# kuailehaha/liuzhou

Measured on AMD Instinct MI355X. Metric: self-play positions/sec (fixed sims/move), higher is better.
Workload: dtype f16

## Files before the change

### liuzhou_amd/build.py

```python
from __future__ import annotations

import os
import shutil
import subprocess

PKG = os.path.dirname(os.path.abspath(__file__))
CSRC = os.path.join(PKG, "csrc")
LIB = os.path.join(PKG, "libliuzhou_hip.so")
SOURCES = ("lz_ops.hip", "lz_engine.hip", "lz_net.hip", "lz_net_f32.hip", "lz_train.hip", "lz_search.hip", "lz_symmetry.hip",
           "lz_dedup.hip")
HEADERS = ("lz_rules.h", "lz_soa.h", "lz_symmetry.h", "lz_wave.h", "lz_rng.h", "lz_net_dev.h", "lz_live_index.h", "lz_surprise.h", "lz_tree_dev.h", "lz_dedup.h", os.path.join("..", "..", "include", "liuzhou_hip.h"))


def hipcc_path() -> str:
    for cand in (os.environ.get("HIPCC"), "/opt/rocm/bin/hipcc", shutil.which("hipcc")):
        if cand and os.path.exists(cand):
            return cand
    raise RuntimeError("hipcc not found (expected /opt/rocm/bin/hipcc)")


HOST_LIB = os.path.join(PKG, "libliuzhou_host.so")
HOST_SOURCE = os.path.join(CSRC, "lz_host.cpp")
HOST_SOURCES = (HOST_SOURCE, os.path.join(CSRC, "lz_scalar.cpp"),
                os.path.join(CSRC, "lz_symmetry_host.cpp"),
                os.path.join(CSRC, "lz_dedup_host.cpp"))


def build_host(force: bool = False, verbose: bool = False) -> str:
    deps = list(HOST_SOURCES) + [os.path.join(CSRC, h) for h in HEADERS] + [os.path.join(PKG, "..", "include", "liuzhou_scalar.h")]
    if not force and os.path.exists(HOST_LIB) and all(
            (not os.path.exists(d)) or os.path.getmtime(d) <= os.path.getmtime(HOST_LIB) for d in deps):
        return HOST_LIB
    cxx = os.environ.get("CXX") or shutil.which("g++") or shutil.which("c++")
    if not cxx:
        raise RuntimeError("no host C++ compiler (g++) found for libliuzhou_host.so")
    cmd = [cxx, "-O2", "-std=c++17", "-ffp-contract=off", "-fPIC", "-shared", "-fvisibility=hidden", "-o", HOST_LIB,
           *HOST_SOURCES]
    if verbose:
        print(" ".join(cmd))
    subprocess.check_call(cmd)
    return HOST_LIB


def needs_build() -> bool:
    if not os.path.exists(LIB):
        return True
    t = os.path.getmtime(LIB)
    deps = [os.path.join(CSRC, s) for s in SOURCES if os.path.exists(os.path.join(CSRC, s))]
    deps += [os.path.join(CSRC, h) for h in HEADERS]
    return any(os.path.exists(d) and os.path.getmtime(d) > t for d in deps)


def build_hip(force: bool = False, verbose: bool = False) -> str:
    if not force and not needs_build():
        return LIB
    srcs = [os.path.join(CSRC, s) for s in SOURCES if os.path.exists(os.path.join(CSRC, s))]
    cmd = [hipcc_path(), "--offload-arch=gfx950", "-O3", "-std=c++17", "-ffp-contract=off", "-fPIC", "-shared",
           "-fvisibility=hidden", "-o", LIB] + srcs
    if verbose:
        print(" ".join(cmd))
    subprocess.check_call(cmd)
    return LIB


def build_variant(tag: str, defs, force: bool = True, verbose: bool = False) -> str:
    out = os.path.join(PKG, "_exp", f"liblz_{tag}.so")
    os.makedirs(os.path.dirname(out), exist_ok=True)
    if not force and os.path.exists(out) and os.path.getmtime(out) >= os.path.getmtime(LIB):
        return out
    srcs = [os.path.join(CSRC, s) for s in SOURCES if os.path.exists(os.path.join(CSRC, s))]
    cmd = [hipcc_path(), "--offload-arch=gfx950", "-O3", "-std=c++17", "-ffp-contract=off", "-fPIC", "-shared",
           "-fvisibility=hidden", *[d if d.startswith("-") else "-D" + d for d in defs], "-o", out] + srcs
    if verbose:
        print(" ".join(cmd))
    subprocess.check_call(cmd)
    return out


EXT_SOURCE = os.path.join(CSRC, "v0_core_ext.cpp")
EXT_NAME = "_v0_core_native"


def ext_path() -> str:
    import sysconfig
    return os.path.join(PKG, EXT_NAME + (sysconfig.get_config_var("EXT_SUFFIX") or ".so"))


def build_ext(force: bool = False, verbose: bool = False) -> str:
    out = ext_path()
    deps = [EXT_SOURCE, os.path.join(PKG, "..", "include", "liuzhou_hip.h")]
    if not force and os.path.exists(out) and all(os.path.getmtime(d) <= os.path.getmtime(out) for d in deps):
        return out
    import sysconfig
    import pybind11
    from torch.utils import cpp_extension as ce
    cxx = os.environ.get("CXX") or shutil.which("g++") or shutil.which("c++")
    if not cxx:
        raise RuntimeError("no host C++ compiler (g++) found for the compiled v0_core layer")
    rocm = os.environ.get("ROCM_PATH", "/opt/rocm")
    inc = ["-I" + p for p in ce.include_paths()] + ["-I" + sysconfig.get_paths()["include"], "-I" + pybind11.get_include(),
                                                    "-I" + os.path.join(rocm, "include")]
    libdir = ce.library_paths()[0]
    cmd = [cxx, "-O2", "-std=c++17", "-fPIC", "-shared", "-fvisibility=hidden", "-w", "-D__HIP_PLATFORM_AMD__=1", "-DUSE_ROCM=1",
           "-DTORCH_API_INCLUDE_EXTENSION_H", "-DTORCH_EXTENSION_NAME=" + EXT_NAME, "-D_GLIBCXX_USE_CXX11_ABI=1", *inc,
           "-o", out, EXT_SOURCE, "-L" + libdir, "-Wl,-rpath," + libdir, "-ltorch_python", "-ltorch", "-ltorch_cpu", "-lc10",
           "-lc10_hip", "-ldl", "-lpthread"]
    if verbose:
        print(" ".join(cmd))
    subprocess.check_call(cmd)
    return out


if __name__ == "__main__":
    import sys
    if len(sys.argv) >= 3 and sys.argv[1] == "variant":
        print(build_variant(sys.argv[2], sys.argv[3:], verbose=True))
        sys.exit(0)
    print(build_hip(force=True, verbose=True))
    print(build_host(force=True, verbose=True))
    print(build_ext(force=True, verbose=True))
```

### liuzhou_amd/csrc/lz_engine.hip

```cpp
#include <hip/hip_runtime.h>
#include <hip/amd_detail/amd_hip_unsafe_atomics.h>
#include <math.h>
#include <stdint.h>

#include <mutex>

#include "lz_rng.h"
#include "lz_tree_dev.h"

namespace {

__global__ __launch_bounds__(kBlock) void pack_states_kernel(LzStateSoA s, int64_t B, Packed* __restrict__ out) {
    const int64_t i = (int64_t)blockIdx.x * kBlock + threadIdx.x;
    if (i >= B) return;
    State st;
    st.black = cells_equal(s.board + i * 36, 1);
    st.white = cells_equal(s.board + i * 36, -1);
    st.mb = cells_nonzero(s.marks_black + i * 36);
    st.mw = cells_nonzero(s.marks_white + i * 36);
    st.phase = (int)s.phase[i]; st.player = (int)s.current_player[i];
    st.pm_req = (int)s.pending_marks_required[i]; st.pm_rem = (int)s.pending_marks_remaining[i];
    st.pc_req = (int)s.pending_captures_required[i]; st.pc_rem = (int)s.pending_captures_remaining[i];
    st.forced = (int)s.forced_removals_done[i]; st.move_count = (int)s.move_count[i];
    st.msc = (int)s.moves_since_capture[i];
    out[i] = pack(st);
}

__global__ __launch_bounds__(kBlock) void packed_planes_kernel(const Packed* __restrict__ states, int64_t B,
                                                               float* __restrict__ out) {
    const int lane = lane_id();
    const int64_t g = (int64_t)blockIdx.x * kWavesPerBlock + __builtin_amdgcn_readfirstlane((int)(threadIdx.x >> 6));
    if (g >= B) return;
    const State s = unpack(states[g]);
    const bool blk = s.player == 1;
    const uint64_t own = blk ? s.black : s.white, opp = blk ? s.white : s.black;
    const uint64_t sm = blk ? s.mb : s.mw, om = blk ? s.mw : s.mb;
    float4* orow = reinterpret_cast<float4*>(out + g * 396);
    for (int j = lane; j < 99; j += kWave) {
        const int plane = j / 9, cell0 = (j - plane * 9) * 4;
        uint32_t bits;
        if (plane < 4) {
            const uint64_t src = plane == 0 ? own : plane == 1 ? opp : plane == 2 ? sm : om;
            bits = (uint32_t)(src >> cell0) & 0xFu;
        } else bits = (s.phase == plane - 3) ? 0xFu : 0u;
        orow[j] = make_float4((bits & 1) ? 1.f : 0.f, (bits & 2) ? 1.f : 0.f, (bits & 4) ? 1.f : 0.f, (bits & 8) ? 1.f : 0.f);
    }
}

__global__ __launch_bounds__(kBlock) void tree_begin_kernel(Tree t) {
    const int g = blockIdx.x * kBlock + threadIdx.x;
    if (g >= t.B) return;
    begin_game(t, g);
}


__global__ __launch_bounds__(kBlock) void pos_clear_kernel(int* __restrict__ tab, int64_t n) {
    for (int64_t i = (int64_t)blockIdx.x * kBlock + threadIdx.x; i < n / 4; i += (int64_t)gridDim.x * kBlock)
        reinterpret_cast<int4*>(tab)[i] = make_int4(-1, -1, -1, -1);
}

template <bool FORCED = false, bool GUMBEL = false, bool SOLVER = false, bool SHAPE = false>
__global__ __launch_bounds__(kBlock) void tree_select_kernel(Tree t, ForcedArgs fa, GumbelArgs ga, ShapeArgs sh) {
    const int g = wave_game();
    if (g >= t.B) return;
    tree_select<FORCED, GUMBEL, SOLVER, SHAPE>(t, g, lane_id(), load_root_info(t, g), -1, -1, nullptr, FORCED ? fa.k : 0.0,
                                               fa.count, &ga, GUMBEL, &sh);
}
__global__ __launch_bounds__(kBlock) void gumbel_root_kernel(Tree t, GumbelArgs ga,
                                                             const uint8_t* __restrict__ root_noise) {
    const int g = wave_game();
    if (g >= t.B) return;
    if (root_noise != nullptr && root_noise[g] == 0) return;
    gumbel_root_step(t, g, lane_id(), ga);
}


template <bool IS_ROOT, bool COMPACT = false, bool CAP = false, bool SOLVER = false>
__global__ __launch_bounds__(kBlock) void tree_expand_kernel(Tree t, const float* __restrict__ lp1,
                                                             const float* __restrict__ lp2,
                                                             const float* __restrict__ lpm,
                                                             const float* __restrict__ priors220,
                                                             const float* __restrict__ values,
                                                             const float* __restrict__ noise, int noise_stride,
                                                             float epsilon, int step, CapArrays cap, SolverArgs sv) {
    LZ_EXPAND_SCRATCH(sc);
    const int g = wave_game();
    if (g >= t.B) return;
    ptrdiff_t o = 0;
    if (COMPACT) o = (ptrdiff_t)(t.leaf_kind[g] == kLeafExpand ? t.live_row[g] : 0) - g;
    if (CAP && IS_ROOT && !cap_noise(cap, g)) noise = nullptr;
    tree_expand<IS_ROOT, 0, SOLVER>(t, g, lane_id(), lp1 ? lp1 + o * 36 : nullptr, lp2 ? lp2 + o * 36 : nullptr,
                                    lpm ? lpm + o * 36 : nullptr, priors220 ? priors220 + o * 220 : nullptr, values + o,
                                    noise, noise_stride, epsilon, sc, nullptr, step, nullptr, nullptr, &sv);
}

constexpr int kScanBlock = 1024;
constexpr int kScanUnroll = 8;
__global__ __launch_bounds__(kScanBlock) void tree_live_scan_kernel(Tree t, unsigned long long* __restrict__ count) {
    __shared__ int wave_total[kScanBlock / kWave];
    const int tid = threadIdx.x, lane = tid & (kWave - 1), w = tid / kWave;
    const int rounds = (t.B + kScanBlock - 1) / kScanBlock;
    int cnt = 0;
    for (int r0 = 0; r0 < rounds; r0 += kScanUnroll) {
        int kind[kScanUnroll];
#pragma unroll
        for (int u = 0; u < kScanUnroll; ++u) {
            const int g = (r0 + u) * kScanBlock + tid;
            kind[u] = (r0 + u < rounds && g < t.B) ? t.leaf_kind[g] : kLeafInactive;
        }
#pragma unroll
        for (int u = 0; u < kScanUnroll; ++u) cnt += kind[u] == kLeafExpand ? 1 : 0;
    }
    int incl = cnt;
#pragma unroll
    for (int d = 1; d < kWave; d <<= 1) {
        const int v = __shfl_up(incl, d, kWave);
        if (lane >= d) incl += v;
    }
    if (lane == kWave - 1) wave_total[w] = incl;
    __syncthreads();
    int before = 0, total = 0;
    for (int i = 0; i < kScanBlock / kWave; ++i) { if (i < w) before += wave_total[i]; total += wave_total[i]; }
    int row = before + incl - cnt;
    for (int r0 = 0; r0 < rounds; r0 += kScanUnroll) {
        int kind[kScanUnroll];
        Packed st[kScanUnroll];
#pragma unroll
        for (int u = 0; u < kScanUnroll; ++u) {
            const int g = (r0 + u) * kScanBlock + tid;
            const bool in = r0 + u < rounds && g < t.B;
            kind[u] = in ? t.leaf_kind[g] : kLeafInactive;
            if (in) st[u] = load_state(&t.leaf_state[g]);
        }
#pragma unroll
        for (int u = 0; u < kScanUnroll; ++u) {
            if (kind[u] != kLeafExpand) continue;
            const int g = (r0 + u) * kScanBlock + tid;
            t.live_row[g] = row;
            t.live_state[row] = st[u];
            ++row;
        }
    }
    if (tid == 0) *count = (unsigned long long)total;
}

__global__ __launch_bounds__(kScanBlock) void tree_live_scan_seg_kernel(Tree t, int seg_games, int num_segs,
                                                                        unsigned long long* __restrict__ count,
                                                                        long long* __restrict__ seg_row) {
    __shared__ int wave_total[kScanBlock / kWave];
    const int tid = threadIdx.x, lane = tid & (kWave - 1), w = tid / kWave;
    const int rounds = (seg_games + kScanBlock - 1) / kScanBlock;
    int base = 0, end = 0;
    if (tid == 0) seg_row[0] = 0;
    for (int k = 0; k < num_segs; ++k) {
        const int g0 = k * seg_games;
        int cnt = 0;
        for (int r0 = 0; r0 < rounds; r0 += kScanUnroll) {
            int kind[kScanUnroll];
#pragma unroll
            for (int u = 0; u < kScanUnroll; ++u) {
                const int i = (r0 + u) * kScanBlock + tid;
                kind[u] = (r0 + u < rounds && i < seg_games) ? t.leaf_kind[g0 + i] : kLeafInactive;
            }
#pragma unroll
            for (int u = 0; u < kScanUnroll; ++u) cnt += kind[u] == kLeafExpand ? 1 : 0;
        }
        int incl = cnt;
#pragma unroll
        for (int d = 1; d < kWave; d <<= 1) {
            const int v = __shfl_up(incl, d, kWave);
            if (lane >= d) incl += v;
        }
        if (lane == kWave - 1) wave_total[w] = incl;
        __syncthreads();
        int before = 0, total = 0;
        for (int i = 0; i < kScanBlock / kWave; ++i) { if (i < w) before += wave_total[i]; total += wave_total[i]; }
        __syncthreads();
        int row = base + before + incl - cnt;
        for (int r0 = 0; r0 < rounds; r0 += kScanUnroll) {
            int kind[kScanUnroll];
            Packed st[kScanUnroll];
#pragma unroll
            for (int u = 0; u < kScanUnroll; ++u) {
                const int i = (r0 + u) * kScanBlock + tid;
                const bool in = r0 + u < rounds && i < seg_games;
                kind[u] = in ? t.leaf_kind[g0 + i] : kLeafInactive;
                if (in) st[u] = load_state(&t.leaf_state[g0 + i]);
            }
#pragma unroll
            for (int u = 0; u < kScanUnroll; ++u) {
                if (kind[u] != kLeafExpand) continue;
                const int g = g0 + (r0 + u) * kScanBlock + tid;
                t.live_row[g] = row;
                t.live_state[row] = st[u];
                ++row;
            }
        }
        end = base + total;
        if (tid == 0) seg_row[k + 1] = end;
        base = (end + 15) & ~15;
    }
    if (tid == 0) *count = (unsigned long long)base;
}

template <bool IS_ROOT, bool COMPACT = false, bool CAP = false, bool FORCED = false, bool GUMBEL = false,
          bool SOLVER = false, bool SHAPE = false>
__global__ __launch_bounds__(kBlock) void tree_expand_select_kernel(Tree t, const float* __restrict__ lp1,
                                                                    const float* __restrict__ lp2,
                                                                    const float* __restrict__ lpm,
                                                                    const float* __restrict__ values,
                                                                    const float* __restrict__ noise, int noise_stride,
                                                                    float epsilon, int step, CapArrays cap,
                                                                    ForcedArgs fa, GumbelArgs ga, SolverArgs sv,
                                                                    ShapeArgs sh) {
#ifndef LZ_EXP_NO_TREE_PRIO
    __builtin_amdgcn_s_setprio(3);
#endif
    LZ_EXPAND_SCRATCH(sc);
    const int g = wave_game();
    if (g >= t.B) return;
    const int lane = lane_id();
    RootInfo root;
    ptrdiff_t o = 0;
    if (COMPACT) o = (ptrdiff_t)(t.leaf_kind[g] == kLeafExpand ? t.live_row[g] : 0) - g;
#ifdef LZ_EXP_TREE_STAMPS
    const unsigned long long lz_t0 = __builtin_readcyclecounter();
#endif
    if (CAP && IS_ROOT && !cap_noise(cap, g)) noise = nullptr;
    tree_expand<IS_ROOT, 0, SOLVER>(t, g, lane, lp1 + o * 36, lp2 + o * 36, lpm + o * 36, nullptr, values + o, noise,
                                    noise_stride, epsilon, sc, &root, step, nullptr, nullptr, &sv LZ_TSTAMP_PASS);
    __threadfence_block();
    const bool gum_on = GUMBEL && (!CAP || cap_noise(cap, g));
    if (GUMBEL && IS_ROOT && gum_on) { gumbel_root_step(t, g, lane, ga); __threadfence_block(); }
    if (CAP && cap_spent(cap, g, step)) {
        if (lane == 0) t.leaf_kind[g] = kLeafInactive;
        return;
    }
    if (IS_ROOT) root = load_root_info(t, g);
    LZ_TSTAMP(g, 7)
    const double fk = FORCED && (!CAP || cap_noise(cap, g)) ? fa.k : 0.0;
    tree_select<FORCED, GUMBEL, SOLVER, SHAPE>(t, g, lane, root, -1, -1, nullptr, fk, fa.count, &ga, gum_on, &sh LZ_TSTAMP_PASS);
#ifdef LZ_EXP_TREE_STAMPS
    LZ_TADD(g, 19, 1)
#endif
}

constexpr int kSplitMaxGames = 8192;
template <bool COMPACT, bool CAP = false, bool FORCED = false, bool GUMBEL = false>
__global__ __launch_bounds__(kBlock) void tree_expand_select_split_kernel(Tree t, const float* __restrict__ lp1,
                                                                          const float* __restrict__ lp2,
                                                                          const float* __restrict__ lpm,
                                                                          const float* __restrict__ values, int step,
                                                                          CapArrays cap, ForcedArgs fa, GumbelArgs ga) {
    __builtin_amdgcn_s_setprio(3);
    LZ_EXPAND_SCRATCH(sc);
    __shared__ int s_flag[kWavesPerBlock / 2];
    const int wv = __builtin_amdgcn_readfirstlane((int)(threadIdx.x >> 6));
    const int pair = wv >> 1, role = wv & 1;
    const int g = blockIdx.x * (kWavesPerBlock / 2) + pair;
    const int lane = lane_id();
    if (role == 0 && lane == 0) s_flag[pair] = 0;
    __syncthreads();
    if (g >= t.B) return;
    volatile int* flag = &s_flag[pair];
    ptrdiff_t o = 0;
    if (COMPACT) o = (ptrdiff_t)(t.leaf_kind[g] == kLeafExpand ? t.live_row[g] : 0) - g;
    if (role == 0) {
        tree_expand<false, 1>(t, g, lane, lp1 + o * 36, lp2 + o * 36, lpm + o * 36, nullptr, values + o, nullptr, 0, 0.f, sc,
                              nullptr, step, flag);
        __builtin_amdgcn_fence(__ATOMIC_RELEASE, "workgroup");
        if (lane == 0) *flag = kSplitExpanded;
    } else {
        RootInfo root;
        SplitInfo split;
        tree_expand<false, 2>(t, g, lane, lp1 + o * 36, lp2 + o * 36, lpm + o * 36, nullptr, values + o, nullptr, 0, 0.f, sc,
                              &root, step, flag, &split);
        __threadfence_block();
        split_wait(flag, kSplitInputsRead);
        if (CAP && cap_spent(cap, g, step)) {
            if (lane == 0) t.leaf_kind[g] = kLeafInactive;
            return;
        }
        const double fk = FORCED && (!CAP || cap_noise(cap, g)) ? fa.k : 0.0;
        const bool gum_on = GUMBEL && (!CAP || cap_noise(cap, g));
        tree_select<FORCED, GUMBEL>(t, g, lane, root, split.wait_edge, split.nolegal_edge, flag, fk, fa.count, &ga, gum_on);
    }
}

constexpr int kWaveDepth = 160;
struct WaveArrays {
    int K, cap;
    int* path; int* path_len; int* leaf_kind; Packed* leaf_state; float* leaf_value; int* leaf_edge; int* leaf_parent;
    int* sims_done; int* unfinished;
    int* eval_row; Packed* eval_state; unsigned long long* eval_count;
    unsigned long long* eval_total;
    int max_back;
};
struct Level { int e0, ne_pl, parent_n, node; double last_sc; int last_k, in_edge; };
static_assert(sizeof(Level) == 32, "level record is 32 bytes");

__device__ __forceinline__ Tree slot_view(const Tree& t, const WaveArrays& w, int j) {
    Tree v = t;
    const size_t o = (size_t)j * t.B;
    v.path = w.path + o * w.cap; v.path_cap = w.cap; v.path_len = w.path_len + o; v.leaf_kind = w.leaf_kind + o;
    v.leaf_state = w.leaf_state + o; v.leaf_value = w.leaf_value + o; v.leaf_edge = w.leaf_edge + o;
    v.leaf_parent = w.leaf_parent + o;
    return v;
}

__device__ __forceinline__ void tree_select_wave(const Tree& t, const WaveArrays& w, int g, int lane,
                                                 const RootInfo& root, int sims, Level* stack, int* leaf_node,
                                                 int* leaf_act) {
    const int done = w.sims_done[g];
    int to_collect = sims - done;
    to_collect = to_collect < w.K ? to_collect : w.K;
    const bool live = t.root_terminal[g] == 0 && root.ne > 0 && to_collect > 0;
    const Node* nodes = t.nodes + (size_t)g * t.node_cap;
    const Edge* edges = t.edges;
    int found = 0;
    if (live) {
        int d = 0;
        int e0 = root.e0, ne = root.ne, parent_n = root.visits, node_player = root.player, node = 0;
        double last_sc = INFINITY;
        int last_k = -1;
        Edge mine[2];
        double sc[2] = {0.0, 0.0};
        bool loaded = false;
        int ups = 0;
        bool last_leaf = false;
        while (found < to_collect) {
            if (!loaded) {
                const double sq = sqrt((double)(parent_n > 1 ? parent_n : 1));
#pragma unroll
                for (int r = 0; r < 2; ++r) {
                    const int k = r * kWave + lane;
                    sc[r] = __builtin_nan("");
                    if (k < ne) {
                        mine[r] = load_edge(&edges[(size_t)(e0 + k)]);
                        const int n = edge_n(mine[r].n_info);
                        double q = 0.0;
                        if (n > 0) {
                            const double mv = mine[r].W / (double)n;
                            const int child_player = (edge_info(mine[r].n_info) & kInfoWhite) ? -1 : 1;
                            q = child_player == node_player ? mv : -mv;
                        }
                        const double u = t.c_puct * (double)mine[r].P * sq / (1.0 + (double)n);
                        sc[r] = q + u;
                    }
                }
                loaded = true;
            }
            double best = -INFINITY;
            int best_k = -1;
#pragma unroll
            for (int r = 0; r < 2; ++r) {
                const int k = r * kWave + lane;
                const bool open = sc[r] < last_sc || (sc[r] == last_sc && k > last_k);
                if (open && sc[r] > best) { best = sc[r]; best_k = k; }
            }
            const double mx = lzw::wave_max(best);
            const uint64_t lo = __ballot(best_k >= 0 && best_k < kWave && best == mx);
            int chosen = -1;
            if (lo) chosen = __ffsll((unsigned long long)lo) - 1;
            else {
                const uint64_t hi = __ballot(best_k >= kWave && best == mx);
                if (hi) chosen = kWave + __ffsll((unsigned long long)hi) - 1;
            }
            if (chosen < 0) {
                if (last_leaf && ++ups > w.max_back) break;
                if (d == 0) break;
                if (++ups > w.max_back) break;
                last_leaf = false;
                --d;
                const Level up = stack[d];
                e0 = up.e0; ne = up.ne_pl & 0xFF; node_player = (up.ne_pl & 0x100) ? -1 : 1; parent_n = up.parent_n;
                node = up.node; last_sc = up.last_sc; last_k = up.last_k;
                loaded = false;
                continue;
            }
            chosen = __builtin_amdgcn_readfirstlane(chosen);
            last_sc = mx; last_k = chosen;
            const int src = chosen & 63;
            const bool up2 = chosen >= kWave;
            const uint32_t c_ni = (uint32_t)lzw::lane_bcast((int)(up2 ? mine[1].n_info : mine[0].n_info), src);
            const int c_child = lzw::lane_bcast(up2 ? mine[1].child : mine[0].child, src);
            const int c_begin = lzw::lane_bcast(up2 ? mine[1].cbegin : mine[0].cbegin, src);
            const int c_meta = lzw::lane_bcast((int)(up2 ? mine[1].act : mine[0].act) | ((int)(up2 ? mine[1].cn : mine[0].cn) << 8), src);
            const uint8_t info = edge_info(c_ni);
            const int child_player = (info & kInfoWhite) ? -1 : 1;
            const int edge_id = e0 + chosen;
            const int entry = edge_id | (child_player != node_player ? (int)kPathFlip : 0);
            const bool terminal = (info & kInfoTerminal) != 0;
            if (terminal || c_child < 0) {
                const size_t slot = (size_t)found * t.B + g;
                int* path = w.path + slot * w.cap;
                for (int l = lane; l < d; l += kWave) path[l] = stack[l + 1].in_edge;
                if (lane == 0) {
                    path[d] = entry;
                    w.path_len[slot] = d + 1;
                    w.leaf_kind[slot] = terminal ? kLeafTerminal : kLeafExpand;
                    w.leaf_value[slot] = terminal ? (float)((int)((info >> 2) & 3) - 1) : 0.f;
                    w.leaf_edge[slot] = edge_id;
                    w.leaf_parent[slot] = node;
                    leaf_node[found] = node;
                    leaf_act[found] = terminal ? -1 : (c_meta & 0xFF);
                }
                ++found;
                last_leaf = true;
                continue;
            }
            last_leaf = false;
            if (d + 1 >= kWaveDepth) continue;
            if (lane == 0) {
                Level here;
                here.e0 = e0; here.ne_pl = ne | (node_player < 0 ? 0x100 : 0); here.parent_n = parent_n; here.node = node;
                here.last_sc = last_sc; here.last_k = last_k; here.in_edge = stack[d].in_edge;
                stack[d] = here;
                stack[d + 1].in_edge = entry;
            }
            __builtin_amdgcn_fence(__ATOMIC_RELEASE, "wavefront");
            __builtin_amdgcn_wave_barrier();
            __builtin_amdgcn_fence(__ATOMIC_ACQUIRE, "wavefront");
            ++d;
            e0 = c_begin; ne = c_meta >> 8; parent_n = edge_n(c_ni); node_player = child_player; node = c_child;
            last_sc = INFINITY; last_k = -1;
            loaded = false;
        }
        __builtin_amdgcn_fence(__ATOMIC_RELEASE, "wavefront");
        __builtin_amdgcn_wave_barrier();
        __builtin_amdgcn_fence(__ATOMIC_ACQUIRE, "wavefront");
        const int act = lane < found ? leaf_act[lane] : -1;
        const uint64_t need = __ballot(act >= 0);
        if (need) {
            unsigned long long base_row = 0ull;
            if (lane == 0) base_row = atomicAdd(w.eval_count, (unsigned long long)__popcll(need));
            base_row = ((unsigned long long)(uint32_t)__builtin_amdgcn_readfirstlane((int)(base_row >> 32)) << 32) |
                       (unsigned long long)(uint32_t)__builtin_amdgcn_readfirstlane((int)(base_row & 0xFFFFFFFFull));
            if (act >= 0) {
                const int pn = leaf_node[lane];
                State leaf = unpack(pn == 0 ? root.state : load_state(&nodes[pn].state));
                int kd, p, q2, ex;
                index_to_code(leaf.phase, act, kd, p, q2, ex);
                apply_legal(leaf, kd, p, q2);
                const Packed ps = pack(leaf);
                const size_t slot = (size_t)lane * t.B + g;
                const unsigned long long row = base_row + (unsigned long long)__popcll(need & ((1ull << lane) - 1ull));
                w.leaf_state[slot] = ps;
                w.eval_row[slot] = (int)row;
                w.eval_state[row] = ps;
            }
        }
    }
    for (int j = found + lane; j < w.K; j += kWave) w.leaf_kind[(size_t)j * t.B + g] = kLeafInactive;
    if (lane == 0) {
        int nd = done + found;
        if (live && found == 0) nd = sims;
        w.sims_done[g] = nd;
        if (t.root_terminal[g] == 0 && root.ne > 0 && nd < sims) atomicAdd(w.unfinished, 1);
    }
}

__global__ __launch_bounds__(kBlock) void tree_select_wave_kernel(Tree t, WaveArrays w, int sims) {
    __shared__ Level s_stack[kWavesPerBlock][kWaveDepth];
    __shared__ int s_leaf_node[kWavesPerBlock][32], s_leaf_act[kWavesPerBlock][32];
    const int g = wave_game();
    if (g >= t.B) return;
    const int wv = __builtin_amdgcn_readfirstlane((int)(threadIdx.x >> 6));
    __builtin_amdgcn_s_setprio(3);
    tree_select_wave(t, w, g, lane_id(), load_root_info(t, g), sims, s_stack[wv], s_leaf_node[wv], s_leaf_act[wv]);
}

__global__ __launch_bounds__(kBlock) void wave_budget_reset_kernel(WaveArrays w, int B, int reset_done) {
    const int g = blockIdx.x * kBlock + threadIdx.x;
    if (g == 0) { *w.unfinished = 0; *w.eval_total += *w.eval_count; *w.eval_count = 0ull; }
    if (reset_done && g < B) w.sims_done[g] = 0;
}

__global__ __launch_bounds__(kBlock) void tree_expand_wave_kernel(Tree t, WaveArrays w, const float* __restrict__ lp1,
                                                                  const float* __restrict__ lp2,
                                                                  const float* __restrict__ lpm,
                                                                  const float* __restrict__ priors220,
                                                                  const float* __restrict__ values, int slot_major) {
    LZ_EXPAND_SCRATCH(sc);
    const int g = wave_game();
    if (g >= t.B) return;
    const int lane = lane_id();
    __builtin_amdgcn_s_setprio(3);
    uint32_t second = 0;
    for (int pass = 0; pass < 2; ++pass) {
        for (int j = 0; j < w.K; ++j) {
            const size_t slot = (size_t)j * t.B + g;
            bool run;
            if (pass == 0) {
                const int kind = w.leaf_kind[slot];
                if (kind == kLeafInactive) break;
                run = kind == kLeafTerminal;
                if (kind == kLeafExpand) {
                    const State s = unpack(load_state(&w.leaf_state[slot]));
                    if (legal_count(legal_actions(s, 0)) == 0) run = true;
                    else second |= 1u << j;
                }
            } else {
                run = (second >> j) & 1u;
            }
            if (!run) continue;
            const ptrdiff_t o = slot_major ? (ptrdiff_t)j * t.B
                                                     : (ptrdiff_t)(w.leaf_kind[slot] == kLeafExpand ? w.eval_row[slot] : 0) - g;
            tree_expand<false>(slot_view(t, w, j), g, lane, lp1 ? lp1 + o * 36 : nullptr, lp2 ? lp2 + o * 36 : nullptr,
                               lpm ? lpm + o * 36 : nullptr, priors220 ? priors220 + o * 220 : nullptr, values + o,
                               nullptr, 0, 0.f, sc);
            __threadfence_block();
        }
    }
}

constexpr int kMarkWordsMax = 1024;
constexpr int kMarkWordsBig = 8192;

__device__ __forceinline__ void pos_rebuild(const Tree& t, int g, int lane, int kept) {
    if (t.pos_index == nullptr) return;
    int* tab = t.pos_index + (size_t)g * t.pos_slots;
    for (int i = lane; i < t.pos_slots / 4; i += kWave) reinterpret_cast<int4*>(tab)[i] = make_int4(-1, -1, -1, -1);
    __threadfence_block();
    const uint32_t mask = (uint32_t)t.pos_slots - 1u;
    const Node* nodes = t.nodes + (size_t)g * t.node_cap;
    for (int id = 1 + lane; id < kept; id += kWave) {
        const uint32_t h = pos_hash(load_state(&nodes[id].state));
        for (int p = 0; p < kWave; ++p)
            if (atomicCAS(&tab[(h + (uint32_t)p) & mask], -1, id) == -1) break;
    }
}

template <int WPB>
__global__ __launch_bounds__(WPB * kWave) void tree_advance_kernel(Tree t, const int* __restrict__ played_action,
                                                              const uint8_t* __restrict__ reset, int reserve_nodes,
                                                              int mark_words, int* __restrict__ dropped,
                                                              int* __restrict__ pruned, long long* __restrict__ ticks) {
    extern __shared__ uint64_t s_adv[];
    const int lane = lane_id();
    const int wv = __builtin_amdgcn_readfirstlane((int)(threadIdx.x >> 6));
    const int g = blockIdx.x * WPB + wv;
    if (g >= t.B) return;
    Node* nodes = t.nodes + (size_t)g * t.node_cap;
    Edge* edges = t.edges;
    uint64_t* mark = s_adv + (size_t)wv * mark_words;
    int* nprefix = reinterpret_cast<int*>(s_adv + (size_t)WPB * mark_words) + (size_t)wv * mark_words;
    const uint64_t lt = (1ull << lane) - 1ull;
    auto rank_of = [&](int id) { return nprefix[id >> 6] + __popcll(mark[id >> 6] & ((1ull << (id & 63)) - 1ull)); };

    const Packed rs = t.root_state[g];
    const bool act = t.active == nullptr || t.active[g] != 0;
    const int ne = nodes[0].nedges, e0 = nodes[0].edge_begin;
    const int played = played_action != nullptr ? played_action[g] : -1;
    int c = -1, new_n = 0;
    double new_w = 0.0;
    if (act && !(reset != nullptr && reset[g]) && !t.root_terminal[g] && ne > 0 && played >= 0) {
        int found = -1;
#pragma unroll
        for (int r = 0; r < 2; ++r) {
            const int k = r * kWave + lane;
            const uint64_t hit = __ballot(k < ne && (int)edges[(size_t)(e0 + (k < ne ? k : 0))].act == played);
            if (found < 0 && hit) found = r * kWave + __ffsll((unsigned long long)hit) - 1;
        }
        if (found >= 0) {
            const Edge E = edges[(size_t)(e0 + found)];
            if (E.child > 0 && !(edge_info(E.n_info) & kInfoTerminal)) {
                const Packed cs = nodes[E.child].state;
                if (cs.w0 == rs.w0 && cs.w1 == rs.w1 && cs.w2 == rs.w2 && cs.w3 == rs.w3) {
                    c = E.child; new_n = edge_n(E.n_info); new_w = E.W;
                }
            }
        }
    }
    const int nn = t.n_nodes[g];
    const int words = (nn + 63) >> 6;
    int kept_nodes = 0;
    if (ticks != nullptr && lane == 0) { ticks[(size_t)g * 8] = (long long)wall_clock64(); ticks[(size_t)g * 8 + 4] = nn; }
    if (c > 0 && words > mark_words) {
        c = -1;
        if (lane == 0 && dropped != nullptr) atomicAdd(dropped, 1);
    }
    if (c > 0) {
        const int node_budget = t.node_cap - reserve_nodes;
        bool cut = false;
        constexpr int kAhead = 4;
        for (int w0 = 0; w0 < words && !cut; w0 += kAhead) {
            int par[kAhead];
#pragma unroll
// ... 1549 lines not shown
```

### liuzhou_amd/csrc/lz_search.hip

```cpp
#include <hip/hip_runtime.h>
#include <math.h>
#include <stdint.h>
#include <stdlib.h>

#include "../../include/liuzhou_hip.h"
#include "lz_net_dev.h"
#include "lz_tree_dev.h"

namespace {

constexpr int kCuSlots = 4096;

__device__ __forceinline__ int cu_key() {
    const unsigned hw = __builtin_amdgcn_s_getreg((4 ) | (8 << 6) | ((8 - 1) << 11));
    const unsigned xcc = __builtin_amdgcn_s_getreg((20 ) | (0 << 6) | ((4 - 1) << 11));
    return (int)(((xcc & 15u) << 8) | (hw & 255u)) & (kCuSlots - 1);
}

struct SearchArgs {
    int sims;
    const float* noise; int noise_stride; float epsilon;
    int* cu_slots;
    int stagger_ticks;
    long long* phase_ticks;
    int exp_mode;
};

template <int C, int S, int W>
__global__ __launch_bounds__(W * 64, 2) void tree_search_persistent_kernel(NetParams P, Tree t, SearchArgs a, float* lp1,
                                                                           float* lp2, float* lpm, float* values) {
    static_assert(S % W == 0, "every wave owns the same number of games");
    constexpr int GPW = S / W;
    extern __shared__ __attribute__((aligned(16))) unsigned char lds[];
    NetCtx<C, S, W> ctx;
    net_setup<C, S, W>(P, lds, ctx);
    const int g0 = blockIdx.x * S;
    const int nvalid = (t.B - g0) < S ? (t.B - g0) : S;
    int slot = 0;
    if (a.cu_slots != nullptr) {
        __shared__ int s_slot;
        if (threadIdx.x == 0) s_slot = atomicAdd(&a.cu_slots[cu_key()], 1);
        __syncthreads();
        slot = __builtin_amdgcn_readfirstlane(s_slot);
        if (a.stagger_ticks > 0 && __builtin_amdgcn_readfirstlane((int)(threadIdx.x >> 6)) == 0 && (slot & 1)) {
            const uint64_t t0 = wall_clock64();
            while ((long long)(wall_clock64() - t0) < (long long)a.stagger_ticks) __builtin_amdgcn_s_sleep(64);
        }
    }
    long long tk_net = 0, tk_tree = 0;
    for (int s = 0; s <= a.sims; ++s) {
        const uint64_t c0 = a.phase_ticks != nullptr ? wall_clock64() : 0;
        net_pass<C, S, W>(P, lds, ctx, nullptr, reinterpret_cast<const uint64_t*>(t.leaf_state), (int64_t)g0, nvalid, lp1,
                          lp2, lpm, nullptr, values);
        __syncthreads();
        __builtin_amdgcn_fence(__ATOMIC_ACQUIRE, "agent");
        const uint64_t c1 = a.phase_ticks != nullptr ? wall_clock64() : 0;
        if (!(a.exp_mode & 4)) __builtin_amdgcn_s_setprio(3);
        int wave_s = ctx.wave;
        asm volatile("" : "+s"(wave_s));
        static_assert(W * kExpandScratchBytes <= Cfg<C, S, W>::B_BYTES, "expand scratch must fit the dead head region");
        const ExpandScratch sc = {reinterpret_cast<float*>(lds + Cfg<C, S, W>::G_OFF + wave_s * kExpandScratchBytes),
                                  reinterpret_cast<int*>(lds + Cfg<C, S, W>::G_OFF + wave_s * kExpandScratchBytes + 320)};
        if (a.exp_mode & 2) {
            const uint64_t t0 = wall_clock64();
            while ((long long)(wall_clock64() - t0) < 2400) __builtin_amdgcn_s_sleep(16);
        }
#pragma unroll 1
        for (int j = 0; j < GPW; ++j) {
            const int g = g0 + wave_s * GPW + j;
            if (g >= t.B || (a.exp_mode & 3)) break;
            RootInfo root;
            if (s == 0) {
                tree_expand<true>(t, g, ctx.lane, lp1, lp2, lpm, nullptr, values, a.noise, a.noise_stride, a.epsilon, sc, &root, s);
                if (a.sims > 0) {
                    __threadfence_block();
                    root = load_root_info(t, g);
                    tree_select(t, g, ctx.lane, root);
                }
            } else {
                tree_expand<false>(t, g, ctx.lane, lp1, lp2, lpm, nullptr, values, nullptr, 0, 0.f, sc, &root, s);
                if (s < a.sims) {
                    __threadfence_block();
                    tree_select(t, g, ctx.lane, root);
                }
            }
        }
        if ((a.exp_mode & 8) ? (((slot + s) & 1) != 0) : ((a.exp_mode & 16) ? ((slot & 1) != 0) : false))
            __builtin_amdgcn_s_setprio(1);
        else
            __builtin_amdgcn_s_setprio(0);
        if (a.phase_ticks != nullptr) {
            asm volatile("s_waitcnt vmcnt(0) lgkmcnt(0)" ::: "memory");
            const uint64_t c2 = wall_clock64();
            tk_net += (long long)(c1 - c0); tk_tree += (long long)(c2 - c1);
        }
    }
    if (a.phase_ticks != nullptr && threadIdx.x == 0) {
        a.phase_ticks[4 * blockIdx.x] = tk_net;
        a.phase_ticks[4 * blockIdx.x + 1] = tk_tree;
        a.phase_ticks[4 * blockIdx.x + 2] = slot;
        a.phase_ticks[4 * blockIdx.x + 3] = cu_key();
    }
}

__global__ void zero_i32_kernel(int* p, int n) {
    for (int i = threadIdx.x; i < n; i += blockDim.x) p[i] = 0;
}

template <int C, int S, int W>
int configure_search() {
    return hipFuncSetAttribute(reinterpret_cast<const void*>(tree_search_persistent_kernel<C, S, W>),
                               hipFuncAttributeMaxDynamicSharedMemorySize, Cfg<C, S, W>::LDS_BYTES) == hipSuccess
               ? LZ_OK : LZ_ERR_LAUNCH;
}

bool g_search_configured[64] = {};

}

extern "C" int lz_prof_mark_begin(void* stream);
extern "C" int lz_prof_mark_end(void* stream, int64_t evals);

extern "C" {

int lz_tree_search_persistent(const LzTreeDesc* d, const LzNetDesc* net, int64_t sims, float* lp1, float* lp2,
                              float* lpmc, float* values, const float* noise, int64_t noise_stride, float epsilon,
                              int continue_trees, int32_t* cu_slots, int64_t stagger_us, int64_t* phase_ticks,
                              void* stream) {
    if (!tree_ok(d) || !net || sims < 0 || !lp1 || !lp2 || !lpmc || !values || stagger_us < 0) return LZ_ERR_ARG;
    if (cap_set(d)) return LZ_ERR_UNSUPPORTED;
    if (kld_set(d)) return LZ_ERR_UNSUPPORTED;
    if (forced_set(d)) return LZ_ERR_UNSUPPORTED;
    if (gumbel_set(d)) return LZ_ERR_UNSUPPORTED;
    if (solver_set(d)) return LZ_ERR_UNSUPPORTED;
    if (shape_set(d)) return LZ_ERR_UNSUPPORTED;
    if (!net->wfrag || !net->fparams) return LZ_ERR_ARG;
    if (net->blocks < 0 || net->blocks > 15 || net->num_layers != 2 + 2 * net->blocks) return LZ_ERR_ARG;
    if ((reinterpret_cast<uintptr_t>(net->wfrag) & 15) || (reinterpret_cast<uintptr_t>(net->fparams) & 15)) return LZ_ERR_ALIGN;
    if (net->channels != 64 || (net->flags & (4 | 8))) return LZ_ERR_UNSUPPORTED;
    const int64_t B = d->num_games;
    if (B == 0) return LZ_OK;
    int device = 0;
    if (hipGetDevice(&device) != hipSuccess || device < 0 || device >= 64) return LZ_ERR_LAUNCH;
    if (!g_search_configured[device]) {
        const int rc = configure_search<64, 8, 4>();
        if (rc) return rc;
        g_search_configured[device] = true;
    }
    int rc = continue_trees ? LZ_OK : lz_tree_begin(d, stream);
    if (rc) return rc;
    hipStream_t stm = as_stream(stream);
    if (cu_slots != nullptr)
        hipLaunchKernelGGL(zero_i32_kernel, dim3(1), dim3(256), 0, stm, cu_slots, kCuSlots);
    const NetParams P = make_net_params(net);
    SearchArgs a;
    a.sims = (int)sims; a.noise = noise; a.noise_stride = (int)noise_stride; a.epsilon = epsilon;
    a.cu_slots = cu_slots;
    a.stagger_ticks = (int)((stagger_us > 10000 ? 10000 : stagger_us) * 100);
    a.phase_ticks = reinterpret_cast<long long*>(phase_ticks);
    a.exp_mode = 0;
#ifdef LZ_EXP_SEARCH_MODES
    a.exp_mode = getenv("LZ_EXP_SEARCH_MODE") ? atoi(getenv("LZ_EXP_SEARCH_MODE")) : 0;
#endif
    using K = Cfg<64, 8, 4>;
    const unsigned grid = (unsigned)((B + 8 - 1) / 8);
    (void)lz_prof_mark_begin(stream);
    hipLaunchKernelGGL((tree_search_persistent_kernel<64, 8, 4>), dim3(grid), dim3(K::THREADS), K::LDS_BYTES, stm, P,
                       no_share(make_tree(d)), a, lp1, lp2, lpmc, values);
    (void)lz_prof_mark_end(stream, B * (sims + 1));
    return st();
}

int lz_tree_search_persistent_grid(int64_t num_games) { return (int)((num_games + 7) / 8); }

}
```

### liuzhou_amd/csrc/lz_tree_dev.h

```cpp
#pragma once
#include <hip/hip_runtime.h>
#include <hip/amd_detail/amd_hip_unsafe_atomics.h>
#include <math.h>
#include <stdint.h>

#include "lz_rng.h"
#include "lz_soa.h"
#include "lz_symmetry.h"
#include "lz_wave.h"

using namespace lz;

namespace {

constexpr int kWave = 64;
constexpr int kBlock = 256;
constexpr int kWavesPerBlock = 4;
constexpr int kMaxChildren = 72;

enum LeafKind : int { kLeafInactive = 0, kLeafExpand = 1, kLeafTerminal = 2, kLeafReusedRoot = 3, kLeafShared = 4 };
constexpr uint8_t kInfoWhite = 1;
constexpr uint8_t kInfoTerminal = 2;
constexpr uint8_t kInfoProven = 16;
constexpr uint8_t kInfoDecided = kInfoTerminal | kInfoProven;

struct Edge {
    double W;
    float P;
    uint32_t n_info;
    int32_t child;
    int32_t cbegin;
    uint8_t act;
    uint8_t cn;
    uint8_t pad[6];
};
static_assert(sizeof(Edge) == 32, "edge record is 32 bytes");
struct Node {
    Packed state;
    int32_t edge_begin, nedges;
    int32_t parent;
    int32_t old_begin;
};
static_assert(sizeof(Node) == 48, "node record is 48 bytes");
__device__ __forceinline__ int edge_n(uint32_t ni) { return (int)(ni & 0xFFFFFFu); }
__device__ __forceinline__ uint8_t edge_info(uint32_t ni) { return (uint8_t)(ni >> 24); }

struct Tree {
    int B, node_cap, chunk, path_cap, chunk_cap;
    const Packed* root_state;
    Node* nodes; Edge* edges;
    int* n_nodes; int* n_edges;
    int* chunk_list; int* n_chunks; int* free_chunks; int* pool_top;
    int* pool_stats;
    int* root_visits; double* root_W; float* root_init_value;
    int* path; int* path_len; int* leaf_kind; Packed* leaf_state; float* leaf_value;
    uint8_t* root_terminal; const uint8_t* active;
    int* leaf_edge; int* leaf_parent;
    double c_puct;
    int fast_select;
    int* trace_kind; Packed* trace_leaf; float* trace_heads; float* trace_priors; float* trace_value;
    int trace_cap;
    int* eval_count;
    Packed* live_state; int* live_row; unsigned long long* live_count;
    int* pos_index; float* node_value; int* leaf_src; int* share_count;
    int pos_slots, share;
    int* leaf_sym; int* trace_sym; const int* sym_salt; const int64_t* sym_game; const int64_t* sym_ply;
    uint64_t sym_seed; int sym_mode, sym_fixed;
};
struct CapArrays { const int* sim_budget; const uint8_t* root_noise; };
struct ForcedArgs { double k; int* count; };
struct SolverArgs { int* root_proven; int* count; };
struct ShapeArgs { double fpu, fpu_root; const double* table; int flags, table_len; };
constexpr int kShapeFpu = 1, kShapeTable = 2;
constexpr double kShapeFix = 1073741824.0;
struct GumbelArgs {
    double c_visit, c_scale;
    const float* g; const int* table;
    float* gl; int* base; int* root_base; float* root_value; int* count;
    int m, sims, stride;
};

typedef unsigned int u32x4 __attribute__((ext_vector_type(4)));
__device__ __forceinline__ Edge load_edge(const Edge* p) {
    const u32x4* q = reinterpret_cast<const u32x4*>(p);
    union U { u32x4 v[2]; Edge e; __device__ U() {} } u;
    u.v[0] = q[0]; u.v[1] = q[1];
    return u.e;
}
__device__ __forceinline__ Packed load_state(const Packed* p) {
    const u32x4* q = reinterpret_cast<const u32x4*>(p);
    union U { u32x4 v[2]; Packed s; __device__ U() {} } u;
    u.v[0] = q[0]; u.v[1] = q[1];
    return u.s;
}
constexpr uint32_t kPathFlip = 0x80000000u;

__device__ __forceinline__ int lane_id() { return threadIdx.x & 63; }
__device__ __forceinline__ int wave_game() {
    return blockIdx.x * kWavesPerBlock + __builtin_amdgcn_readfirstlane((int)(threadIdx.x >> 6));
}
__device__ __forceinline__ bool same_state(const Packed& a, const Packed& b) {
    return a.w0 == b.w0 && a.w1 == b.w1 && a.w2 == b.w2 && a.w3 == b.w3;
}
__device__ __forceinline__ uint32_t pos_hash(const Packed& s) {
    uint64_t h = s.w0 * 0x9E3779B97F4A7C15ull;
    h = (h ^ (h >> 29) ^ s.w1) * 0xBF58476D1CE4E5B9ull;
    h = (h ^ (h >> 31) ^ s.w2) * 0x94D049BB133111EBull;
    h = (h ^ (h >> 27) ^ s.w3) * 0x9E3779B97F4A7C15ull;
    return (uint32_t)(h >> 32);
}
struct PosWindow { int entry; int first_empty; uint32_t base; };
__device__ __forceinline__ PosWindow pos_window(const Tree& t, int g, const Packed& s, int nn, int lane) {
    const int* tab = t.pos_index + (size_t)g * t.pos_slots;
    const uint32_t mask = (uint32_t)t.pos_slots - 1u;
    PosWindow w;
    w.base = pos_hash(s) & mask;
    w.entry = tab[(w.base + (uint32_t)lane) & mask];
    const uint64_t em = __ballot(w.entry < 1 || w.entry >= nn);
    w.first_empty = em ? __ffsll((unsigned long long)em) - 1 : kWave;
    return w;
}
__device__ __forceinline__ int pos_find(const Tree& t, int g, const Packed& s, int nn, int lane) {
    const PosWindow w = pos_window(t, g, s, nn, lane);
    bool hit = false;
    if (lane < w.first_empty) hit = same_state(load_state(&t.nodes[(size_t)g * t.node_cap + w.entry].state), s);
    const uint64_t hm = __ballot(hit);
    return hm ? lzw::lane_bcast(w.entry, __ffsll((unsigned long long)hm) - 1) : -1;
}

#ifdef LZ_EXP_TREE_STAMPS
__device__ unsigned long long g_tree_stamps[32];
#define LZ_TSTAMP_ON(g) ((g) == 5)
#define LZ_TSTAMP(g, k) if (LZ_TSTAMP_ON(g)) { asm volatile("s_waitcnt vmcnt(0) lgkmcnt(0)" ::: "memory"); \
        if (lane_id() == 0) { atomicAdd(&g_tree_stamps[k], (unsigned long long)__builtin_readcyclecounter() - lz_t0); \
                              atomicAdd(&g_tree_stamps[20 + (k)], 1ull); } }
#define LZ_TSTAMP_ARG , unsigned long long lz_t0 = 0
#define LZ_TSTAMP_PASS , lz_t0
#define LZ_TCLOCK(g, var) unsigned long long var = 0; if (LZ_TSTAMP_ON(g)) { asm volatile("s_waitcnt vmcnt(0) lgkmcnt(0)" ::: "memory"); var = __builtin_readcyclecounter(); }
#define LZ_TADD(g, k, v) if (LZ_TSTAMP_ON(g) && lane_id() == 0) atomicAdd(&g_tree_stamps[k], (unsigned long long)(v));
#else
#define LZ_TSTAMP(g, k)
#define LZ_TCLOCK(g, var)
#define LZ_TADD(g, k, v)
#define LZ_TSTAMP_ARG
#define LZ_TSTAMP_PASS
#endif

constexpr uint32_t kPurposeSymmetry = 3;
__device__ __forceinline__ int leaf_sym_for(const Tree& t, int g, const Packed& leaf) {
    if (t.sym_mode == 1) return t.sym_fixed & 7;
    const uint64_t game = (uint64_t)t.sym_game[g];
    const lzrng::U4 c = {(uint32_t)game, (uint32_t)(game >> 32) ^ (uint32_t)t.sym_salt[g],
                         (uint32_t)t.sym_ply[g] ^ (kPurposeSymmetry << 30), pos_hash(leaf)};
    return (int)(lzrng::philox4x32_10(c, (uint32_t)t.sym_seed, (uint32_t)(t.sym_seed >> 32)).x >> 29);
}

__device__ __forceinline__ double terminal_value_for_mover(const State& s) {
    const int st = game_status(s);
    if (st == 1 || st == -1) return st == s.player ? 1.0 : -1.0;
    return 0.0;
}


__device__ __forceinline__ bool cap_spent(const CapArrays& c, int g, int step) {
    return c.sim_budget != nullptr && step >= c.sim_budget[g];
}
__device__ __forceinline__ bool cap_noise(const CapArrays& c, int g) {
    return c.root_noise == nullptr || c.root_noise[g] != 0;
}

__device__ __forceinline__ void release_chunks(const Tree& t, int g, int keep) {
    const int nc = t.n_chunks[g];
    if (nc > keep) {
        const int base = atomicAdd(t.pool_top, nc - keep);
        const int* list = t.chunk_list + (size_t)g * t.chunk_cap;
        for (int i = keep; i < nc; ++i) t.free_chunks[base + (i - keep)] = list[i];
    }
    t.n_chunks[g] = keep < nc ? keep : nc;
}
__device__ __forceinline__ void release_chunks_wave(const Tree& t, int g, int keep, int lane) {
    const int nc = t.n_chunks[g];
    if (nc > keep) {
        int base = 0;
        if (lane == 0) base = atomicAdd(t.pool_top, nc - keep);
        base = __builtin_amdgcn_readfirstlane(base);
        const int* list = t.chunk_list + (size_t)g * t.chunk_cap;
        for (int i = keep + lane; i < nc; i += kWave) t.free_chunks[base + (i - keep)] = list[i];
        if (lane == 0) t.n_chunks[g] = keep;
    }
}
__device__ __forceinline__ bool root_pending(const Tree& t, int g) {
    return t.n_nodes[g] == 1 && t.nodes[(size_t)g * t.node_cap].nedges < 0 && t.root_terminal[g] == 0;
}

__device__ __forceinline__ int take_chunk(const Tree& t, int g, bool for_root = false) {
    const int nc = t.n_chunks[g];
    if (nc >= t.chunk_cap) { atomicAdd(t.pool_stats, 1); return -1; }
    const int top = atomicSub(t.pool_top, 1) - 1;
    const int reserved = for_root ? 0 : __atomic_load_n(t.pool_stats + 2, __ATOMIC_RELAXED);
    if (top < reserved) { atomicAdd(t.pool_top, 1); atomicAdd(t.pool_stats, 1); return -1; }
    if (for_root && root_pending(t, g)) atomicSub(t.pool_stats + 2, 1);
    atomicMin(t.pool_stats + 1, top);
    const int cid = t.free_chunks[top];
    t.chunk_list[(size_t)g * t.chunk_cap + nc] = cid;
    t.n_chunks[g] = nc + 1;
    return cid * t.chunk;
}

__device__ __forceinline__ void begin_game(const Tree& t, int g, bool release = true) {
    const bool was_pending = root_pending(t, g);
    if (release) release_chunks(t, g, 0);
    const Packed rs = t.root_state[g];
    Node& root = t.nodes[(size_t)g * t.node_cap];
    root.state = rs;
    root.edge_begin = 0;
    root.nedges = -1;
    root.parent = -1;
    t.n_nodes[g] = 1;
    t.n_edges[g] = 0;
    t.root_visits[g] = 0;
    t.root_W[g] = 0.0;
    t.root_init_value[g] = 0.f;
    t.path_len[g] = 0;
    const State s = unpack(rs);
    const bool act = t.active == nullptr || t.active[g] != 0;
    const bool term = game_status(s) != 0;
    t.root_terminal[g] = (term || !act) ? 1 : 0;
    t.leaf_kind[g] = (term || !act) ? kLeafInactive : kLeafExpand;
    const bool pending = !(term || !act);
    if (pending != was_pending) atomicAdd(t.pool_stats + 2, pending ? 1 : -1);
    t.leaf_state[g] = rs;
    t.leaf_value[g] = 0.f;
    if (t.sym_mode != 0) {
        const int k = pending ? leaf_sym_for(t, g, rs) : 0;
        t.leaf_sym[g] = k;
        if (k != 0) t.leaf_state[g] = sym_packed(k, rs);
    }
}

struct RootInfo { int ne, e0, visits, player; Packed state; };
__device__ __forceinline__ RootInfo load_root_info(const Tree& t, int g) {
    RootInfo r;
    const Node* root = t.nodes + (size_t)g * t.node_cap;
    r.state = load_state(&root->state);
    r.ne = root->nedges; r.e0 = root->edge_begin;
    r.visits = t.root_visits[g];
    r.player = ((r.state.w0 >> 53) & 1) ? -1 : 1;
    return r;
}

constexpr int kSplitInputsRead = 1, kSplitExpanded = 2;
__device__ __forceinline__ void split_wait(volatile int* flag, int phase) {
    while (*flag < phase) __builtin_amdgcn_s_sleep(1);
    __builtin_amdgcn_fence(__ATOMIC_ACQUIRE, "workgroup");
}

__device__ __forceinline__ double gumbel_bfly(double v) {
#pragma unroll
    for (int o = 32; o > 0; o >>= 1) v += __shfl_xor(v, o);
    return v;
}
struct GumbelLane { double score[2], sigma[2], vmix; int L[2]; };
__device__ __forceinline__ GumbelLane gumbel_scores(const GumbelArgs& ga, int g, int lane, const int (&n)[2],
                                                    const float (&P)[2], const double (&q)[2], const bool (&ok)[2]) {
    const bool vis0 = ok[0] && n[0] > 0, vis1 = ok[1] && n[1] > 0;
    const double p0 = vis0 ? (double)P[0] : 0.0, p1 = vis1 ? (double)P[1] : 0.0;
    const double pq0 = vis0 ? (double)P[0] * q[0] : 0.0, pq1 = vis1 ? (double)P[1] * q[1] : 0.0;
    const double Pv = gumbel_bfly(p0 + p1), Pq = gumbel_bfly(pq0 + pq1);
    const int T = lzw::lane_bcast(lzw::wave_incl_scan((ok[0] ? n[0] : 0) + (ok[1] ? n[1] : 0)), kWave - 1);
    const int nl = ok[1] && n[1] > n[0] ? n[1] : (ok[0] ? n[0] : 0);
    const double nmax = (double)lzw::wave_max((float)nl);
    const double v0 = (double)ga.root_value[g];
    const double tm = (double)T;
    GumbelLane o;
    o.vmix = (T == 0 || Pv <= 0.0) ? v0 : (v0 + tm * (Pq / Pv)) / (1.0 + tm);
    const double scale = (ga.c_visit + nmax) * ga.c_scale;
#pragma unroll
    for (int r = 0; r < 2; ++r) {
        const int k = r * kWave + lane;
        const bool in = ok[r] && k < ga.stride;
        const float gl = in ? ga.gl[(size_t)g * ga.stride + k] : -INFINITY;
        const int n0 = in ? ga.base[(size_t)g * ga.stride + k] : 0;
        const double cq = (ok[r] && n[r] > 0) ? q[r] : o.vmix;
        o.sigma[r] = scale * (0.5 * cq);
        o.score[r] = (double)gl + o.sigma[r];
        o.L[r] = (ok[r] ? n[r] : 0) - n0;
    }
    return o;
}
__device__ __forceinline__ int gumbel_argmax(const GumbelLane& s, const bool (&cand)[2], int lane) {
    double best = -INFINITY;
    int best_k = -1;
#pragma unroll
    for (int r = 0; r < 2; ++r)
        if (cand[r] && (best_k < 0 || s.score[r] > best)) { best = s.score[r]; best_k = r * kWave + lane; }
    const double mx = lzw::wave_max(best_k >= 0 ? best : -INFINITY);
    const uint64_t lo = __ballot(best_k >= 0 && best_k < kWave && best == mx);
    if (lo) return __ffsll((unsigned long long)lo) - 1;
    const uint64_t hi = __ballot(best_k >= kWave && best == mx);
    return hi ? kWave + __ffsll((unsigned long long)hi) - 1 : -1;
}
__device__ __forceinline__ void gumbel_root_step(const Tree& t, int g, int lane, const GumbelArgs& ga) {
    if (t.root_terminal[g]) return;
    const int kind = t.leaf_kind[g];
    if (kind != kLeafExpand && kind != kLeafReusedRoot) return;
    const Node* root = t.nodes + (size_t)g * t.node_cap;
    const int ne = root->nedges, e0 = root->edge_begin;
    if (ne <= 0) return;
#pragma unroll
    for (int r = 0; r < 2; ++r) {
        const int k = r * kWave + lane;
        if (k < ne && k < ga.stride) {
            const Edge e = load_edge(&t.edges[(size_t)e0 + k]);
            ga.gl[(size_t)g * ga.stride + k] = ga.g[(size_t)g * ga.stride + k] + logf(e.P);
            ga.base[(size_t)g * ga.stride + k] = edge_n(e.n_info);
        }
    }
    if (lane == 0) {
        const int rv = t.root_visits[g];
        ga.root_base[g] = rv;
        ga.root_value[g] = kind == kLeafReusedRoot ? (rv > 0 ? (float)(t.root_W[g] / (double)rv) : 0.f)
                                                   : t.root_init_value[g];
        if (ga.count != nullptr) ga.count[g] += 1;
    }
}

__device__ __forceinline__ int solver_x(uint8_t info, int owner_player) {
    const int d = (int)((info >> 2) & 3) - 1;
    return ((info & kInfoWhite) ? -1 : 1) == owner_player ? d : -d;
}
__device__ __forceinline__ int solver_rule(const uint8_t (&info)[2], const bool (&ok)[2], int owner_player) {
    bool win = false, open = false, draw = false;
#pragma unroll
    for (int r = 0; r < 2; ++r) {
        if (!ok[r]) continue;
        const bool dec = (info[r] & kInfoDecided) != 0;
        const int x = solver_x(info[r], owner_player);
        win = win || (dec && x > 0);
        draw = draw || (dec && x == 0);
        open = open || !dec;
    }
    if (__ballot(win)) return 3;
    if (__ballot(open)) return 0;
    return __ballot(draw) ? 2 : 1;
}
__device__ __forceinline__ int solver_root_rule(const Tree& t, const RootInfo& root, int lane) {
    uint8_t inf[2]; bool ok[2];
#pragma unroll
    for (int r = 0; r < 2; ++r) {
        const int k = r * kWave + lane;
        ok[r] = k < root.ne;
        inf[r] = ok[r] ? edge_info(t.edges[(size_t)(root.e0 + k)].n_info) : (uint8_t)0;
    }
    return solver_rule(inf, ok, root.player);
}
__device__ __forceinline__ int solver_climb(const Tree& t, int g, int lane, const SolverArgs& sv, const int* path, int j,
                                            int e_j, uint8_t info_j, const RootInfo& root) {
    Edge* edges = t.edges;
    int marks = 0;
    while (true) {
        int ye0, yne, yplayer, e_up = -1;
        uint8_t in_info = 0;
        if (j == 0) { ye0 = root.e0; yne = root.ne; yplayer = root.player; }
        else {
            e_up = (int)((uint32_t)path[j - 1] & ~kPathFlip);
            const Edge up = load_edge(&edges[(size_t)e_up]);
            in_info = edge_info(up.n_info);
            if ((in_info & kInfoDecided) || up.child < 0) break;
            ye0 = up.cbegin; yne = up.cn; yplayer = (in_info & kInfoWhite) ? -1 : 1;
        }
        uint8_t inf[2]; bool ok[2];
#pragma unroll
        for (int r = 0; r < 2; ++r) {
            const int k = r * kWave + lane;
            ok[r] = k < yne;
            inf[r] = ok[r] ? edge_info(edges[(size_t)(ye0 + k)].n_info) : (uint8_t)0;
            if (ok[r] && ye0 + k == e_j) inf[r] = info_j;
        }
        const int p = solver_rule(inf, ok, yplayer);
        if (p == 0) break;
        if (j == 0) {
            int fresh = 0;
            if (lane == 0 && sv.root_proven[g] == 0) { sv.root_proven[g] = p; fresh = 1; }
            marks += __builtin_amdgcn_readfirstlane(fresh);
            break;
        }
        const uint8_t mark = (uint8_t)(kInfoProven | ((p - 1) << 2));
        if (lane == 0) atomicOr(&edges[(size_t)e_up].n_info, (uint32_t)mark << 24);
        info_j = (uint8_t)(in_info | mark);
        e_j = e_up;
        ++marks;
        --j;
    }
    return marks;
}

template <bool FORCED = false, bool GUMBEL = false, bool SOLVER = false, bool SHAPE = false>
__device__ __forceinline__ void tree_select(const Tree& t, int g, int lane, const RootInfo& root, int wait_edge = -1,
                                            int nolegal_edge = -1, volatile int* flag = nullptr, double forced_k = 0.0,
                                            int* forced_count = nullptr, const GumbelArgs* gum = nullptr,
                                            bool gum_on = false, const ShapeArgs* sh = nullptr LZ_TSTAMP_ARG) {
    static_assert(!(SHAPE && GUMBEL), "the Gumbel root search has no shaped form");
    if (t.root_terminal[g]) { if (lane == 0) t.leaf_kind[g] = kLeafInactive; return; }
    double node_W = 0.0, init_v = 0.0;
    if (SHAPE && (sh->flags & kShapeFpu)) { node_W = t.root_W[g]; init_v = (double)t.root_init_value[g]; }
    const Node* nodes = t.nodes + (size_t)g * t.node_cap;
    const Edge* edges = t.edges;
    int* path = t.path + (size_t)g * t.path_cap;
    int node = 0, depth = 0;
    int parent_n = root.visits;
    int node_player = root.player;
    int ne = root.ne, e0 = root.e0;
    Packed node_state = root.state;
    int kind = kLeafInactive;
    float term_value = 0.f;
    int leaf_action = 0, leaf_edge = -1;
    while (ne > 0) {
        LZ_TCLOCK(g, lv_t0)
        const Edge* run = edges + (size_t)__builtin_amdgcn_readfirstlane(e0);
        Edge mine[2];
        mine[1] = Edge{};
#pragma unroll
        for (int r = 0; r < 2; ++r) {
            if (r == 1 && ne <= kWave) break;
            const int k = r * kWave + lane;
            if (k < ne) mine[r] = load_edge(&run[k]);
        }
        double c_level = t.c_puct;
        if (SHAPE && (sh->flags & kShapeTable))
            c_level = sh->table[parent_n < sh->table_len - 1 ? (parent_n > 0 ? parent_n : 0) : sh->table_len - 1];
#ifdef LZ_EXP_TREE_STAMPS
        if (LZ_TSTAMP_ON(g)) { LZ_TCLOCK(g, lv_t1) LZ_TADD(g, 16, lv_t1 - lv_t0) lv_t0 = lv_t1; }
#endif
        int chosen = -1;
        if (FORCED && depth == 0 && forced_k > 0.0) {
            bool due[2] = {false, false};
#pragma unroll
            for (int r = 0; r < 2; ++r) {
                if (r == 1 && ne <= kWave) break;
                if (r * kWave + lane < ne) {
                    const double n = (double)edge_n(mine[r].n_info);
                    due[r] = n > 0.0 && n * n < (forced_k * (double)mine[r].P) * (double)parent_n;
                }
            }
            const uint64_t lo = __ballot(due[0]);
            if (lo) chosen = __ffsll((unsigned long long)lo) - 1;
            else if (ne > kWave) {
                const uint64_t hi = __ballot(due[1]);
                if (hi) chosen = kWave + __ffsll((unsigned long long)hi) - 1;
            }
            if (chosen >= 0 && forced_count != nullptr && lane == 0) forced_count[g] += 1;
        }
        if (GUMBEL && depth == 0 && gum_on) {
            int n[2]; float P[2]; double q[2]; bool ok[2];
#pragma unroll
            for (int r = 0; r < 2; ++r) {
                ok[r] = (r == 0 || ne > kWave) && r * kWave + lane < ne;
                n[r] = ok[r] ? edge_n(mine[r].n_info) : 0;
                P[r] = ok[r] ? mine[r].P : 0.f;
                q[r] = 0.0;
                if (n[r] > 0) {
                    const double mv = mine[r].W / (double)n[r];
                    const int child_player = (edge_info(mine[r].n_info) & kInfoWhite) ? -1 : 1;
                    q[r] = child_player == node_player ? mv : -mv;
                }
            }
            const GumbelLane s = gumbel_scores(*gum, g, lane, n, P, q, ok);
            const int started = parent_n - gum->root_base[g];
            const int col = started < 0 ? 0 : (started < gum->sims ? started : gum->sims - 1);
            const int cv = gum->table[(size_t)(gum->m < ne ? gum->m : ne) * gum->sims + col];
            bool cand[2] = {ok[0] && s.L[0] == cv, ok[1] && s.L[1] == cv};
            if (__ballot(cand[0] || cand[1]) == 0ull) { cand[0] = ok[0]; cand[1] = ok[1]; }
            chosen = gumbel_argmax(s, cand, lane);
            if (chosen < 0) break;
        }
        if (!SOLVER && !SHAPE && (!FORCED || chosen < 0) && (!GUMBEL || chosen < 0) && t.fast_select) {
            const float sqf = sqrtf((float)(parent_n > 1 ? parent_n : 1));
            const float cf = (float)t.c_puct;
            float fs[2] = {-INFINITY, -INFINITY};
            bool off_scale = false;
#pragma unroll
            for (int r = 0; r < 2; ++r) {
                if (r == 1 && ne <= kWave) break;
                if (r * kWave + lane < ne) {
                    const int n = edge_n(mine[r].n_info);
                    float q = 0.f;
                    if (n > 0) {
                        const float mv = (float)mine[r].W / (float)n;
                        const int child_player = (edge_info(mine[r].n_info) & kInfoWhite) ? -1 : 1;
                        q = child_player == node_player ? mv : -mv;
                        off_scale = off_scale || !(fabsf(mv) <= 1.0001f);
                    }
                    const float s = q + cf * mine[r].P * sqf / (1.0f + (float)n);
                    fs[r] = s == s ? s : -INFINITY;
                }
            }
            const float b = fs[1] > fs[0] ? fs[1] : fs[0];
            const float m1 = lzw::wave_max_nonan(b);
            const uint64_t w0 = __ballot(fs[0] == m1), w1 = __ballot(fs[1] == m1);
            if (m1 > -INFINITY && m1 < INFINITY && __popcll(w0) + __popcll(w1) == 1 && __ballot(off_scale) == 0ull) {
                const int c = w0 ? __ffsll((unsigned long long)w0) - 1 : kWave + __ffsll((unsigned long long)w1) - 1;
                const float b2 = (c & 63) == lane ? (c < kWave ? fs[1] : fs[0]) : b;
                const float m2 = lzw::wave_max_nonan(b2);
                if (m1 - m2 > 1e-4f * (1.0f + fabsf(m1))) chosen = c;
            }
        }
        bool cand[2] = {true, true};
        if (SOLVER && chosen < 0) {
            bool win[2] = {false, false}, lose[2] = {false, false};
#pragma unroll
            for (int r = 0; r < 2; ++r) {
                if (r == 1 && ne <= kWave) break;
                const uint8_t inf = edge_info(mine[r].n_info);
                if (r * kWave + lane < ne && (inf & kInfoDecided)) {
                    const int x = solver_x(inf, node_player);
                    win[r] = x > 0; lose[r] = x < 0;
                }
            }
            const uint64_t wl = __ballot(win[0]);
            if (wl) chosen = __ffsll((unsigned long long)wl) - 1;
            else if (ne > kWave) {
                const uint64_t wh = __ballot(win[1]);
                if (wh) chosen = kWave + __ffsll((unsigned long long)wh) - 1;
            }
            if (chosen < 0 && __ballot((lane < ne && !lose[0]) || (kWave + lane < ne && !lose[1])) != 0ull) {
                cand[0] = !lose[0]; cand[1] = !lose[1];
            }
        }
        if (chosen < 0) {
            const double sq = sqrt((double)(parent_n > 1 ? parent_n : 1));
            double fpu_q = 0.0;
            if (SHAPE && (sh->flags & kShapeFpu)) {
                bool fresh = false;
                uint64_t s = 0;
#pragma unroll
                for (int r = 0; r < 2; ++r) {
                    if (r == 1 && ne <= kWave) break;
                    if (r * kWave + lane < ne) {
                        const bool dec = SOLVER && (edge_info(mine[r].n_info) & kInfoDecided) != 0;
                        if (edge_n(mine[r].n_info) > 0) s += (uint64_t)((double)mine[r].P * kShapeFix);
                        else fresh = fresh || (!dec && (!SOLVER || cand[r]));
                    }
                }
                if (__ballot(fresh) != 0ull) {
                    const int s0 = lzw::lane_bcast(lzw::wave_incl_scan((int)(s & 0xFFFFFu)), kWave - 1);
                    const int s1 = lzw::lane_bcast(lzw::wave_incl_scan((int)((s >> 20) & 0xFFFFFu)), kWave - 1);
                    const int s2 = lzw::lane_bcast(lzw::wave_incl_scan((int)(s >> 40)), kWave - 1);
                    const uint64_t S = (uint64_t)(uint32_t)s0 + ((uint64_t)(uint32_t)s1 << 20) + ((uint64_t)(uint32_t)s2 << 40);
                    const double V = parent_n > 0 ? node_W / (double)parent_n : init_v;
                    const double red = (depth == 0 ? sh->fpu_root : sh->fpu) * sqrt((double)S / kShapeFix);
                    fpu_q = V - red;
                    if (fpu_q < -1.0) fpu_q = -1.0;
                }
            }
            double best = -INFINITY;
            int best_k = -1;
#pragma unroll
            for (int r = 0; r < 2; ++r) {
                if (r == 1 && ne <= kWave) break;
                const int k = r * kWave + lane;
                if (k < ne && (!SOLVER || cand[r])) {
                    const int n = edge_n(mine[r].n_info);
                    double q = 0.0;
                    if (SOLVER && (edge_info(mine[r].n_info) & kInfoDecided)) {
                        q = (double)solver_x(edge_info(mine[r].n_info), node_player);
                    } else if (n > 0) {
                        const double mv = mine[r].W / (double)n;
                        const int child_player = (edge_info(mine[r].n_info) & kInfoWhite) ? -1 : 1;
                        q = child_player == node_player ? mv : -mv;
                    } else if (SHAPE) {
                        q = fpu_q;
                    }
                    const double u = (SHAPE ? c_level : t.c_puct) * (double)mine[r].P * sq / (1.0 + (double)n);
                    const double sc = q + u;
                    if (sc > best) { best = sc; best_k = k; }
                }
            }
            const double mx = lzw::wave_max(best);
            const uint64_t lo = __ballot(best_k >= 0 && best_k < kWave && best == mx);
            if (lo) chosen = __ffsll((unsigned long long)lo) - 1;
            else {
                const uint64_t hi = __ballot(best_k >= kWave && best == mx);
                if (!hi) break;
                chosen = kWave + __ffsll((unsigned long long)hi) - 1;
            }
        }
        chosen = __builtin_amdgcn_readfirstlane(chosen);
        const int src = chosen & 63;
        const bool up = chosen >= kWave;
        const uint32_t c_ni = (uint32_t)lzw::lane_bcast((int)(up ? mine[1].n_info : mine[0].n_info), src);
        int c_child = lzw::lane_bcast(up ? mine[1].child : mine[0].child, src);
        int c_begin = lzw::lane_bcast(up ? mine[1].cbegin : mine[0].cbegin, src);
        int c_meta = lzw::lane_bcast((int)(up ? mine[1].act : mine[0].act) | ((int)(up ? mine[1].cn : mine[0].cn) << 8), src);
        uint8_t info = edge_info(c_ni);
        if (e0 + chosen == wait_edge) {
            split_wait(flag, kSplitExpanded);
            const Edge fresh = load_edge(&run[chosen]);
            c_child = fresh.child; c_begin = fresh.cbegin;
            c_meta = (int)fresh.act | ((int)fresh.cn << 8);
        }
        if (e0 + chosen == nolegal_edge) info |= kInfoTerminal;
        const int child_player = (info & kInfoWhite) ? -1 : 1;
#ifdef LZ_EXP_TREE_STAMPS
        { LZ_TCLOCK(g, lv_t2) LZ_TADD(g, 17, lv_t2 - lv_t0) LZ_TADD(g, 18, 1) }
#endif
        leaf_edge = e0 + chosen;
        if (lane == 0) path[depth] = leaf_edge | (child_player != node_player ? (int)kPathFlip : 0);
        ++depth;
        if (info & (SOLVER ? kInfoDecided : kInfoTerminal)) {
            kind = kLeafTerminal;
            term_value = (float)((int)((info >> 2) & 3) - 1);
            break;
        }
        if (c_child < 0) { kind = kLeafExpand; leaf_action = c_meta & 0xFF; break; }
        node_state = load_state(&nodes[c_child].state);
        if (SHAPE && (sh->flags & kShapeFpu)) {
            const double w = up ? mine[1].W : mine[0].W;
            node_W = __hiloint2double(lzw::lane_bcast(__double2hiint(w), src), lzw::lane_bcast(__double2loint(w), src));
        }
        parent_n = edge_n(c_ni);
        node_player = child_player;
        node = c_child;
        e0 = c_begin;
        ne = c_meta >> 8;
        if (depth >= t.path_cap - 1) break;
    }
    LZ_TSTAMP(g, 8)
    Packed leaf_packed{};
    int src = -1;
    if (kind == kLeafExpand) {
        State leaf = unpack(node_state);
        int kd, p, q2, ex;
        index_to_code(leaf.phase, leaf_action, kd, p, q2, ex);
        apply_legal(leaf, kd, p, q2);
        leaf_packed = pack(leaf);
        if (t.share) {
            src = pos_find(t, g, leaf_packed, t.n_nodes[g], lane);
            if (src > 0) kind = kLeafShared;
        }
    }
    int sym = 0;
    if (t.sym_mode != 0 && kind == kLeafExpand) {
        sym = __builtin_amdgcn_readfirstlane(leaf_sym_for(t, g, leaf_packed));
        leaf_packed = sym_packed_wave(sym, leaf_packed, lane);
    }
    if (lane == 0) {
        t.path_len[g] = depth;
        t.leaf_kind[g] = kind;
        t.leaf_value[g] = term_value;
        t.leaf_edge[g] = leaf_edge;
        t.leaf_parent[g] = node;
        if (kind == kLeafExpand || kind == kLeafShared) t.leaf_state[g] = leaf_packed;
        if (kind == kLeafShared) t.leaf_src[g] = src;
        if (t.sym_mode != 0) t.leaf_sym[g] = sym;
    }
    LZ_TSTAMP(g, 9)
}

struct ExpandScratch { float* val; int* act; };
constexpr int kExpandScratchBytes = 80 * 8;
#define LZ_EXPAND_SCRATCH(name)                                                            \
    __shared__ float name##_val[kWavesPerBlock][80];                                      \
    __shared__ int name##_act[kWavesPerBlock][80];                                        \
    const int name##_wv = __builtin_amdgcn_readfirstlane((int)(threadIdx.x >> 6));        \
    const ExpandScratch name = {name##_val[name##_wv], name##_act[name##_wv]}

struct SplitInfo { int wait_edge, nolegal_edge; };
template <bool IS_ROOT, int ROLE = 0, bool SOLVER = false>
__device__ __forceinline__ void tree_expand(const Tree& t, int g, int lane, const float* __restrict__ lp1,
                                            const float* __restrict__ lp2, const float* __restrict__ lpm,
                                            const float* __restrict__ priors220, const float* __restrict__ values,
                                            const float* __restrict__ noise, int noise_stride, float epsilon,
                                            ExpandScratch sc, RootInfo* root_after = nullptr, int step = -1,
                                            volatile int* flag = nullptr, SplitInfo* split = nullptr,
                                            const SolverArgs* sv = nullptr LZ_TSTAMP_ARG) {
    static_assert(ROLE == 0 || !IS_ROOT, "the root step is never split");
    static_assert(ROLE == 0 || !SOLVER, "the solver runs on the one-wave step");
    LZ_TSTAMP(g, 0)
    const int kind = t.leaf_kind[g];
    Node* nodes = t.nodes + (size_t)g * t.node_cap;
    Edge* edges = t.edges;
    const int* path = t.path + (size_t)g * t.path_cap;
    RootInfo root{};
    int plen_ld = 0, leaf_edge = -1, leaf_parent = 0, nn_ld = 0, ne_ld = 0, path_entry = 0;
    double root_w = 0.0;
    float leaf_value_ld = 0.f, value_ld = 0.f;
    Packed leaf_packed = t.leaf_state[g];
    const int sym = (t.sym_mode != 0 && kind == kLeafExpand) ? (__builtin_amdgcn_readfirstlane(t.leaf_sym[g]) & 7) : 0;
    if (!IS_ROOT) {
        root = load_root_info(t, g);
        plen_ld = t.path_len[g];
        leaf_edge = t.leaf_edge[g];
        leaf_parent = t.leaf_parent[g];
        path_entry = lane < t.path_cap ? path[lane] : 0;
        root_w = t.root_W[g];
        leaf_value_ld = t.leaf_value[g];
    }
    nn_ld = t.n_nodes[g];
    ne_ld = t.n_edges[g];
    const Packed eval_packed = leaf_packed;
    if (sym != 0) leaf_packed = sym_packed_wave(sym_inverse(sym), eval_packed, lane);
    const bool shared = !IS_ROOT && ROLE == 0 && kind == kLeafShared;
    value_ld = shared ? 0.f : values[g];
    const bool indexed = !IS_ROOT && ROLE != 2 && t.pos_index != nullptr;
    PosWindow pw{0, kWave, 0u};
    if (indexed) pw = pos_window(t, g, leaf_packed, nn_ld, lane);
    int src_begin = 0;
    if (shared) {
        const int src = t.leaf_src[g];
        value_ld = t.node_value[(size_t)g * t.node_cap + src];
        src_begin = nodes[src].edge_begin;
    }
    if (root_after != nullptr) *root_after = root;
    if (ROLE == 1) {
        asm volatile("s_waitcnt vmcnt(0)" ::: "memory");
        if (lane == 0) *flag = kSplitInputsRead;
    }
    if (ROLE == 2) { split->wait_edge = -1; split->nolegal_edge = -1; }
    LZ_TSTAMP(g, 1)
    const bool tracing = ROLE != 2 && t.trace_kind != nullptr && step >= 0 && step < t.trace_cap;
    const size_t tslot = tracing ? (size_t)step * (size_t)t.B + (size_t)g : 0;
    if (tracing) {
        if (lane == 0) {
            t.trace_kind[tslot] = kind; t.trace_leaf[tslot] = eval_packed; t.trace_value[tslot] = value_ld;
            if (t.trace_sym != nullptr) t.trace_sym[tslot] = sym;
        }
        for (int a = lane; a < 220; a += kWave) t.trace_priors[tslot * 220 + a] = 0.f;
    }
    if (kind == kLeafInactive) return;
    if (kind == kLeafReusedRoot) {
        if (IS_ROOT && noise != nullptr) {
            const int ne = nodes[0].nedges, e0 = nodes[0].edge_begin;
            if (ne > 1) {
                const float keep = (float)(1.0 - (double)epsilon);
                float pr[2]; bool ok[2];
#pragma unroll
                for (int r = 0; r < 2; ++r) {
                    const int k = r * kWave + lane;
                    ok[r] = k < ne;
                    pr[r] = ok[r] ? keep * edges[(size_t)(e0 + k)].P + epsilon * noise[(size_t)g * noise_stride + k] : 0.f;
                }
                float psum = 0.f;
#pragma unroll
                for (int r = 0; r < 2; ++r) {
                    uint64_t m = __ballot(ok[r]);
                    while (m) {
                        const int l = __builtin_amdgcn_readfirstlane(__ffsll((unsigned long long)m) - 1);
                        psum += lzw::lane_bcast(pr[r], l);
                        m &= m - 1;
                    }
                }
                const float denom = psum < 1e-8f ? 1e-8f : psum;
#pragma unroll
                for (int r = 0; r < 2; ++r)
                    if (ok[r]) edges[(size_t)(e0 + r * kWave + lane)].P = pr[r] / denom;
            }
        }
        if (SOLVER && IS_ROOT) {
            const RootInfo kept = load_root_info(t, g);
            const int p = kept.ne > 0 ? solver_root_rule(t, kept, lane) : 0;
            if (p != 0 && lane == 0) {
                sv->root_proven[g] = p;
                if (sv->count != nullptr) sv->count[g] += 1;
            }
        }
        return;
    }
    const int plen = IS_ROOT ? 0 : plen_ld;
    double backup_value = 0.0;
    int sol = 0;
    bool sol_terminal = false;
    int leaf_player = 1;

    if (kind == kLeafTerminal) {
        backup_value = (double)leaf_value_ld;
    } else {
        if (shared) { if (t.share_count != nullptr && lane == 0) t.share_count[g] += 1; }
        else if (ROLE != 2 && t.eval_count != nullptr && lane == 0) t.eval_count[g] += 1;
        const State s = unpack(leaf_packed);
        const Legal L = legal_actions(s, 0);
        const int n = legal_count(L);
        leaf_player = s.player;
        if (ROLE == 2) {
            backup_value = n == 0 ? -1.0 : (double)value_ld;
            if (n == 0) split->nolegal_edge = leaf_edge; else split->wait_edge = leaf_edge;
        } else if (n == 0) {
            backup_value = -1.0;
            if (lane == 0) {
                if (IS_ROOT) {
                    if (root_pending(t, g)) atomicSub(t.pool_stats + 2, 1);
                    nodes[0].nedges = 0; t.root_terminal[g] = 1; t.root_init_value[g] = -1.f;
                }
                else atomicOr(&edges[(size_t)leaf_edge].n_info, (uint32_t)kInfoTerminal << 24);
            }
            if (SOLVER && !IS_ROOT) { sol = 1; sol_terminal = true; }
        } else {
            float h1 = 0.f, h2 = 0.f, hm = 0.f;
            const bool heads = priors220 == nullptr;
            if (heads && lane < kCells && !shared) {
                const int hc = sym != 0 ? sym_cell(sym, lane) : lane;
                h1 = lp1[(size_t)g * 36 + hc]; h2 = lp2[(size_t)g * 36 + hc]; hm = lpm[(size_t)g * 36 + hc];
                if (tracing) {
                    float* th = t.trace_heads + tslot * 108;
                    th[hc] = h1; th[36 + hc] = h2; th[72 + hc] = hm;
                }
            }
            float val[4]; int slot[4]; bool lg[4];
            int base = 0;
            float mx = -INFINITY;
#pragma unroll
            for (int it = 0; it < 4; ++it) {
                const int a = it * kWave + lane;
                lg[it] = a < 217 && legal_bit(L, a);
                val[it] = 0.f; slot[it] = 0;
                const uint64_t bal = __ballot(lg[it]);
                if (bal == 0) continue;
                slot[it] = base + __popcll(bal & ((1ull << lane) - 1ull));
                base += __popcll(bal);
                int from = 0, dest = 0, cell = 0;
                if (a >= 36 && a < 180) { from = (a - 36) >> 2; dest = move_dest(from, (a - 36) & 3); dest = dest < 0 ? 0 : (dest > 35 ? 35 : dest); }
                else if (a >= 180 && a < 216) cell = a - 180;
                else if (a < 36) cell = a;
                float x;
                if (heads) {
                    const float p1d = __shfl(h1, dest), p2f = __shfl(h2, from), p1c = __shfl(h1, cell), pmc = __shfl(hm, cell);
                    x = a < 36 ? p1c : a < 180 ? (p2f + p1d) : a < 216 ? pmc : 0.f;
                } else {
                    x = lg[it] ? priors220[(size_t)g * 220 + (sym != 0 ? (int)kSym.action[sym][a] : a)] : 0.f;
                }
                val[it] = x;
                if (heads && lg[it]) mx = fmaxf(mx, x);
            }
            if (heads) {
                mx = lzw::wave_max(mx);
                float sum = 0.f;
#pragma unroll
                for (int it = 0; it < 4; ++it) { val[it] = lg[it] ? expf(val[it] - mx) : 0.f; sum += val[it]; }
                sum = lzw::wave_sum(sum);
#pragma unroll
                for (int it = 0; it < 4; ++it) val[it] = val[it] / sum;
            }
            if (tracing) {
#pragma unroll
                for (int it = 0; it < 4; ++it)
                    if (lg[it]) t.trace_priors[tslot * 220 + it * kWave + lane] = val[it];
            }
            if (IS_ROOT && noise != nullptr && n > 1) {
                const float keep = (float)(1.0 - (double)epsilon);
#pragma unroll
                for (int it = 0; it < 4; ++it)
                    if (lg[it]) val[it] = keep * val[it] + epsilon * noise[(size_t)g * noise_stride + slot[it]];
            }
            LZ_TSTAMP(g, 2)
#pragma unroll
            for (int it = 0; it < 4; ++it)
                if (lg[it]) { sc.val[slot[it]] = val[it]; sc.act[slot[it]] = it * kWave + lane; }
            __builtin_amdgcn_fence(__ATOMIC_RELEASE, "wavefront");
            __builtin_amdgcn_wave_barrier();
            __builtin_amdgcn_fence(__ATOMIC_ACQUIRE, "wavefront");
            float cval[2]; int cact[2];
#pragma unroll
            for (int r = 0; r < 2; ++r) {
                const int k = r * kWave + lane;
                cval[r] = k < n ? sc.val[k] : 0.f;
                cact[r] = k < n ? sc.act[k] : 0;
            }
            float psum = 0.f;
            if (shared) {
#pragma unroll
                for (int r = 0; r < 2; ++r) {
                    const int k = r * kWave + lane;
                    cval[r] = k < n ? edges[(size_t)(src_begin + k)].P : 0.f;
                }
                psum = 1.f;
            } else {
#pragma unroll 4
                for (int k = 0; k < n; ++k) psum += lzw::lane_bcast(k < kWave ? cval[0] : cval[1], k & 63);
            }
            const bool bad = !(psum > 0.f) || !isfinite(psum);
            LZ_TSTAMP(g, 3)
            int node_id = 0, e0 = 0;
            if (lane == 0) {
                e0 = ne_ld;
                const int off = e0 & (t.chunk - 1);
                if (off == 0 || off + n > t.chunk) e0 = take_chunk(t, g, IS_ROOT);
                if (e0 >= 0) {
                    t.n_edges[g] = e0 + n;
                    if (IS_ROOT) node_id = 0;
                    else {
                        node_id = nn_ld; t.n_nodes[g] = node_id + 1;
                        Edge& in = edges[(size_t)leaf_edge];
                        in.child = node_id; in.cbegin = e0; in.cn = (uint8_t)n;
                        nodes[node_id].state = leaf_packed;
                        nodes[node_id].parent = leaf_parent;
                        if (t.node_value != nullptr) t.node_value[(size_t)g * t.node_cap + node_id] = value_ld;
                        if (indexed && !shared && pw.first_empty < kWave)
                            t.pos_index[(size_t)g * t.pos_slots + ((pw.base + (uint32_t)pw.first_empty) & ((uint32_t)t.pos_slots - 1u))] = node_id;
                    }
                    nodes[node_id].edge_begin = e0;
                    nodes[node_id].nedges = n;
                }
                if (IS_ROOT) t.root_init_value[g] = value_ld;
            }
            e0 = __builtin_amdgcn_readfirstlane(e0);
            node_id = __builtin_amdgcn_readfirstlane(node_id);
            const int n_write = e0 >= 0 ? n : 0;
            LZ_TSTAMP(g, 4)
            Edge* new_run = edges + (size_t)(e0 >= 0 ? e0 : 0);
            uint8_t new_info[2] = {0, 0};
            for (int r = 0; r < (n_write > kWave ? 2 : 1); ++r) {
                const int k = r * kWave + lane;
                if (k >= n_write) continue;
                const int a = r == 0 ? cact[0] : cact[1];
                State c = s;
                int kd, p, q2, ex;
                index_to_code(s.phase, a, kd, p, q2, ex);
                apply_legal(c, kd, p, q2);
                uint8_t info = c.player < 0 ? kInfoWhite : 0;
                if (game_status(c) != 0) {
                    const int tv = (int)terminal_value_for_mover(c);
                    info |= kInfoTerminal | (uint8_t)((tv + 1) << 2);
                }
                if (SOLVER) { if (r == 0) new_info[0] = info; else new_info[1] = info; }
                Edge rec;
                rec.W = 0.0;
                rec.P = shared ? (r == 0 ? cval[0] : cval[1]) : bad ? (1.0f / (float)n) : ((r == 0 ? cval[0] : cval[1]) / psum);
                rec.n_info = (uint32_t)info << 24;
                rec.child = -1;
                rec.cbegin = 0;
                rec.act = (uint8_t)a;
                rec.cn = 0;
                rec.pad[0] = rec.pad[1] = rec.pad[2] = rec.pad[3] = rec.pad[4] = rec.pad[5] = 0;
                new_run[k] = rec;
            }
            backup_value = (double)value_ld;
            LZ_TSTAMP(g, 5)
            if (SOLVER && n_write > 0) {
                const bool nok[2] = {lane < n_write, kWave + lane < n_write};
                sol = solver_rule(new_info, nok, s.player);
            }
        }
    }
    if (SOLVER && IS_ROOT && sol != 0 && lane == 0) {
        sv->root_proven[g] = sol;
        if (sv->count != nullptr) sv->count[g] += 1;
    }
    if (IS_ROOT || ROLE == 1) return;
    if (plen > 0) {
        int flips_above = 0;
        for (int hi = plen; hi > 0; hi -= kWave) {
            const int lo = hi > kWave ? hi - kWave : 0;
            const int j = lo + lane;
            const bool in = j < hi;
            const uint32_t pe = !in ? 0u : (lo == 0 ? (uint32_t)path_entry : (uint32_t)path[j]);
            const uint64_t F = __ballot(in && (pe & kPathFlip) != 0u);
            const int above = in ? __popcll(F >> (lane + 1)) : 0;
            if (in) {
                Edge* e = &edges[(size_t)(pe & ~kPathFlip)];
                const double v = ((above + flips_above) & 1) ? -backup_value : backup_value;
                atomicAdd(&e->n_info, 1u);
                unsafeAtomicAdd(&e->W, v);
            }
            flips_above += __popcll(F);
        }
        root.visits += 1;
        if (lane == 0) {
            t.root_visits[g] = root.visits;
            t.root_W[g] = root_w + ((flips_above & 1) ? -backup_value : backup_value);
        }
        if (root_after != nullptr) root_after->visits = root.visits;
        if (SOLVER && sol != 0) {
            const uint8_t mark = (uint8_t)(kInfoProven | ((sol - 1) << 2));
            if (!sol_terminal && lane == 0) atomicOr(&edges[(size_t)leaf_edge].n_info, (uint32_t)mark << 24);
            const uint8_t info_j = (uint8_t)((leaf_player < 0 ? kInfoWhite : 0) | (sol_terminal ? kInfoTerminal : mark));
            const int marks = 1 + solver_climb(t, g, lane, *sv, path, plen - 1, leaf_edge, info_j, root);
            if (sv->count != nullptr && lane == 0) sv->count[g] += marks;
            __builtin_amdgcn_fence(__ATOMIC_ACQ_REL, "agent");
        }
    }
    LZ_TSTAMP(g, 6)
}

inline hipStream_t as_stream(void* s) { return reinterpret_cast<hipStream_t>(s); }
inline int st() { return hipGetLastError() == hipSuccess ? LZ_OK : LZ_ERR_LAUNCH; }

Tree make_tree(const LzTreeDesc* d) {
    Tree t;
    t.B = (int)d->num_games; t.node_cap = d->node_cap; t.chunk = d->edge_chunk; t.path_cap = d->path_cap;
    t.chunk_cap = d->chunk_cap;
    t.chunk_list = d->chunk_list; t.n_chunks = d->n_chunks; t.free_chunks = d->free_chunks; t.pool_top = d->pool_top;
    t.pool_stats = d->pool_stats;
    t.root_state = reinterpret_cast<const Packed*>(d->root_state);
    t.nodes = reinterpret_cast<Node*>(d->nodes);
    t.edges = reinterpret_cast<Edge*>(d->edges);
    t.n_nodes = d->n_nodes; t.n_edges = d->n_edges; t.root_visits = d->root_visits; t.root_W = d->root_w;
    t.root_init_value = d->root_init_value;
    t.path = d->path; t.path_len = d->path_len; t.leaf_kind = d->leaf_kind;
    t.leaf_state = reinterpret_cast<Packed*>(d->leaf_state); t.leaf_value = d->leaf_value;
    t.root_terminal = d->root_terminal; t.active = d->active;
    t.leaf_edge = d->leaf_edge; t.leaf_parent = d->leaf_parent;
    t.c_puct = d->exploration_weight;
    { const char* e = getenv("LZ_TREE_F32SEL"); t.fast_select = (e && e[0] == '1'); }
    const bool tr = d->trace_cap > 0 && d->trace_kind && d->trace_leaf && d->trace_heads && d->trace_priors && d->trace_value;
    t.trace_kind = tr ? d->trace_kind : nullptr;
    t.trace_leaf = tr ? reinterpret_cast<Packed*>(d->trace_leaf) : nullptr;
    t.trace_heads = tr ? d->trace_heads : nullptr;
    t.trace_priors = tr ? d->trace_priors : nullptr;
    t.trace_value = tr ? d->trace_value : nullptr;
    t.trace_cap = tr ? (int)d->trace_cap : 0;
    t.eval_count = d->eval_count;
    const bool live = d->live_state && d->live_row && d->live_count && d->live_count_cap > 0;
    t.live_state = live ? reinterpret_cast<Packed*>(d->live_state) : nullptr;
    t.live_row = live ? d->live_row : nullptr;
    t.live_count = live ? reinterpret_cast<unsigned long long*>(d->live_count) : nullptr;
    const bool pos = d->pos_index && d->node_value && d->leaf_src && d->pos_slots >= kWave &&
                     (d->pos_slots & (d->pos_slots - 1)) == 0;
    t.pos_index = pos ? d->pos_index : nullptr;
    t.node_value = pos ? d->node_value : nullptr;
    t.leaf_src = pos ? d->leaf_src : nullptr;
    t.pos_slots = pos ? (int)d->pos_slots : 0;
    t.share_count = d->share_count;
    { const char* e = getenv("LZ_TREE_SHARE"); t.share = pos && !tr && !(e && e[0] == '0') ? 1 : 0; }
    const bool sym = d->leaf_sym && ((d->sym_mode == 1 && d->sym_fixed >= 0 && d->sym_fixed < 8) ||
                                     (d->sym_mode == 2 && d->sym_salt && d->sym_game && d->sym_ply));
    t.sym_mode = sym ? d->sym_mode : 0;
    t.sym_fixed = sym ? d->sym_fixed : 0;
    t.leaf_sym = sym ? d->leaf_sym : nullptr;
    t.trace_sym = sym && tr ? d->trace_sym : nullptr;
    t.sym_salt = sym ? d->sym_salt : nullptr;
    t.sym_game = sym ? d->sym_game : nullptr;
    t.sym_ply = sym ? d->sym_ply : nullptr;
    t.sym_seed = d->sym_seed;
    return t;
}
inline Tree no_share(Tree t) { t.share = 0; return t; }
inline bool cap_set(const LzTreeDesc* d) { return d->sim_budget != nullptr || d->root_noise != nullptr; }
inline CapArrays make_cap(const LzTreeDesc* d) { return CapArrays{d->sim_budget, d->root_noise}; }
inline bool forced_set(const LzTreeDesc* d) { return d->forced_k > 0.0; }
inline ForcedArgs make_forced(const LzTreeDesc* d) { return ForcedArgs{d->forced_k, d->forced_count}; }
inline bool gumbel_set(const LzTreeDesc* d) { return d->gumbel_m != 0; }
inline bool solver_set(const LzTreeDesc* d) { return d->solver != 0; }
inline int solver_check(const LzTreeDesc* d) { return solver_set(d) && !d->root_proven ? LZ_ERR_ARG : LZ_OK; }
inline SolverArgs make_solver(const LzTreeDesc* d) { return SolverArgs{d->root_proven, d->solver_count}; }
inline bool shape_set(const LzTreeDesc* d) { return (d->puct_shape & (kShapeFpu | kShapeTable)) != 0; }
inline int shape_check(const LzTreeDesc* d) {
    if (!shape_set(d)) return LZ_OK;
    if ((d->puct_shape & kShapeTable) && (!d->cpuct_table || d->cpuct_table_len < 2)) return LZ_ERR_ARG;
    if ((d->puct_shape & kShapeFpu) && (!(d->fpu_reduction >= 0.0) || !(d->fpu_root_reduction >= 0.0) ||
                                        !isfinite(d->fpu_reduction) || !isfinite(d->fpu_root_reduction)))
        return LZ_ERR_ARG;
    return gumbel_set(d) ? LZ_ERR_UNSUPPORTED : LZ_OK;
}
inline ShapeArgs make_shape(const LzTreeDesc* d) {
    return ShapeArgs{d->fpu_reduction, d->fpu_root_reduction, d->cpuct_table, d->puct_shape & (kShapeFpu | kShapeTable),
                     d->cpuct_table_len};
}
inline int gumbel_check(const LzTreeDesc* d) {
    if (!gumbel_set(d)) return LZ_OK;
    if (d->gumbel_m < 0 || d->gumbel_m > kMaxChildren || d->gumbel_sims < 1 || d->gumbel_stride < kMaxChildren ||
        d->gumbel_stride > (1 << 20) || !(d->gumbel_c_visit >= 0.0) || !(d->gumbel_c_scale >= 0.0) ||
        !isfinite(d->gumbel_c_visit) || !isfinite(d->gumbel_c_scale) || !d->gumbel_g || !d->gumbel_table ||
        !d->gumbel_gl || !d->gumbel_base || !d->gumbel_root_base || !d->gumbel_root_value)
        return LZ_ERR_ARG;
    return forced_set(d) ? LZ_ERR_UNSUPPORTED : LZ_OK;
}
inline GumbelArgs make_gumbel(const LzTreeDesc* d) {
    return GumbelArgs{d->gumbel_c_visit, d->gumbel_c_scale, d->gumbel_g, d->gumbel_table, d->gumbel_gl, d->gumbel_base,
                      d->gumbel_root_base, d->gumbel_root_value, d->gumbel_count, d->gumbel_m, d->gumbel_sims,
                      (int)d->gumbel_stride};
}
struct KldArgs {
    double theta; int interval, min_sims;
    int* snapshot; int* budget; long long* stops; long long* saved; double* trace;
};
inline bool kld_set(const LzTreeDesc* d) { return d->kld_threshold != 0.0; }
inline int kld_check(const LzTreeDesc* d) {
    if (!kld_set(d)) return LZ_OK;
    if (!(d->kld_threshold > 0.0) || !isfinite(d->kld_threshold) || d->kld_interval < 1 || d->kld_min_sims < 0 ||
        !d->kld_snapshot || !d->kld_budget || d->kld_budget != d->sim_budget)
        return LZ_ERR_ARG;
    return gumbel_set(d) ? LZ_ERR_UNSUPPORTED : LZ_OK;
}
inline KldArgs make_kld(const LzTreeDesc* d) {
    return KldArgs{d->kld_threshold, d->kld_interval, d->kld_min_sims, d->kld_snapshot, d->kld_budget,
                   reinterpret_cast<long long*>(d->kld_stops), reinterpret_cast<long long*>(d->kld_saved), d->kld_trace};
}
bool tree_ok(const LzTreeDesc* d) {
    return d && d->num_games >= 0 && d->node_cap >= 2 && d->path_cap >= 3 &&
           d->edge_chunk >= 128 && (d->edge_chunk & (d->edge_chunk - 1)) == 0 && d->chunk_cap >= 1 &&
           d->pool_chunks >= 1 && (d->pool_chunks + 1) * (int64_t)d->edge_chunk <= (int64_t)1 << 31 &&
           d->pool_chunks >= d->num_games &&
           d->chunk_list && d->n_chunks && d->free_chunks && d->pool_top && d->pool_stats &&
           d->root_state && d->nodes && d->edges && d->n_nodes && d->n_edges &&
           d->root_visits && d->root_w && d->root_init_value && d->path && d->path_len && d->leaf_kind &&
           d->leaf_state && d->leaf_value && d->root_terminal && d->leaf_edge && d->leaf_parent;
}

}
```

Measured before the change: 12370.

## Cut SGPR pressure in tree kernels by re-reading args and parking values in VGPRs

Kernel arguments for features that are compiled out (cap, forced, gumbel, solver, shape) become empty types, so their fields no longer occupy kernarg space or SGPRs. Inside tree_expand and tree_select, the tree descriptor is re-read through an opaque offset instead of being held live across the function. Long-lived scalars such as the root state, path length and leaf edge are parked in VGPRs and brought back with readfirstlane. The fused expand-select kernel is also capped at 102 SGPRs. The aim is to remove SGPR spills and keep occupancy up, at the cost of extra scalar loads and readfirstlane moves.

```diff
diff --git a/liuzhou_amd/build.py b/liuzhou_amd/build.py
--- a/liuzhou_amd/build.py
+++ b/liuzhou_amd/build.py
@@ -9,7 +9,7 @@
 LIB = os.path.join(PKG, "libliuzhou_hip.so")
 SOURCES = ("lz_ops.hip", "lz_engine.hip", "lz_net.hip", "lz_net_f32.hip", "lz_train.hip", "lz_search.hip", "lz_symmetry.hip",
            "lz_dedup.hip")
-HEADERS = ("lz_rules.h", "lz_soa.h", "lz_symmetry.h", "lz_wave.h", "lz_rng.h", "lz_net_dev.h", "lz_live_index.h", "lz_surprise.h", "lz_tree_dev.h", "lz_dedup.h", os.path.join("..", "..", "include", "liuzhou_hip.h"))
+HEADERS = ("lz_rules.h", "lz_soa.h", "lz_symmetry.h", "lz_wave.h", "lz_rng.h", "lz_net_dev.h", "lz_live_index.h", "lz_surprise.h", "lz_tree_dev.h", "lz_tree_args.h", "lz_dedup.h", os.path.join("..", "..", "include", "liuzhou_hip.h"))
 
 
 def hipcc_path() -> str:
diff --git a/liuzhou_amd/csrc/lz_engine.hip b/liuzhou_amd/csrc/lz_engine.hip
--- a/liuzhou_amd/csrc/lz_engine.hip
+++ b/liuzhou_amd/csrc/lz_engine.hip
@@ -60,11 +60,14 @@
 }
 
 template <bool FORCED = false, bool GUMBEL = false, bool SOLVER = false, bool SHAPE = false>
-__global__ __launch_bounds__(kBlock) void tree_select_kernel(Tree t, ForcedArgs fa, GumbelArgs ga, ShapeArgs sh) {
+__global__ __launch_bounds__(kBlock) void tree_select_kernel(Tree t, ArgsIf<FORCED, ForcedArgs> fa,
+                                                             ArgsIf<GUMBEL, GumbelArgs> ga, ArgsIf<SHAPE, ShapeArgs> sh) {
     const int g = wave_game();
     if (g >= t.B) return;
-    tree_select<FORCED, GUMBEL, SOLVER, SHAPE>(t, g, lane_id(), load_root_info(t, g), -1, -1, nullptr, FORCED ? fa.k : 0.0,
-                                               fa.count, &ga, GUMBEL, &sh);
+    const ForcedArgs* fp = args_ptr<ForcedArgs>(fa);
+    tree_select<FORCED, GUMBEL, SOLVER, SHAPE, ArgsViewed>(t, g, lane_id(), load_root_info(t, g), -1, -1, nullptr,
+                                                           FORCED ? fp->k : 0.0, FORCED ? fp->count : nullptr,
+                                                           args_ptr<GumbelArgs>(ga), GUMBEL, args_ptr<ShapeArgs>(sh));
 }
 __global__ __launch_bounds__(kBlock) void gumbel_root_kernel(Tree t, GumbelArgs ga,
                                                              const uint8_t* __restrict__ root_noise) {
@@ -82,16 +85,18 @@
                                                              const float* __restrict__ priors220,
                                                              const float* __restrict__ values,
                                                              const float* __restrict__ noise, int noise_stride,
-                                                             float epsilon, int step, CapArrays cap, SolverArgs sv) {
+                                                             float epsilon, int step, ArgsIf<CAP, CapArrays> cap,
+                                                             ArgsIf<SOLVER, SolverArgs> sv) {
     LZ_EXPAND_SCRATCH(sc);
     const int g = wave_game();
     if (g >= t.B) return;
     ptrdiff_t o = 0;
     if (COMPACT) o = (ptrdiff_t)(t.leaf_kind[g] == kLeafExpand ? t.live_row[g] : 0) - g;
-    if (CAP && IS_ROOT && !cap_noise(cap, g)) noise = nullptr;
-    tree_expand<IS_ROOT, 0, SOLVER>(t, g, lane_id(), lp1 ? lp1 + o * 36 : nullptr, lp2 ? lp2 + o * 36 : nullptr,
-                                    lpm ? lpm + o * 36 : nullptr, priors220 ? priors220 + o * 220 : nullptr, values + o,
-                                    noise, noise_stride, epsilon, sc, nullptr, step, nullptr, nullptr, &sv);
+    if (CAP && IS_ROOT && !cap_noise(*args_ptr<CapArrays>(cap), g)) noise = nullptr;
+    tree_expand<IS_ROOT, 0, SOLVER, ArgsViewed>(t, g, lane_id(), lp1 ? lp1 + o * 36 : nullptr, lp2 ? lp2 + o * 36 : nullptr,
+                                                lpm ? lpm + o * 36 : nullptr, priors220 ? priors220 + o * 220 : nullptr,
+                                                values + o, noise, noise_stride, epsilon, sc, nullptr, step, nullptr, nullptr,
+                                                args_ptr<SolverArgs>(sv));
 }
 
 constexpr int kScanBlock = 1024;
@@ -205,14 +210,19 @@
 
 template <bool IS_ROOT, bool COMPACT = false, bool CAP = false, bool FORCED = false, bool GUMBEL = false,
           bool SOLVER = false, bool SHAPE = false>
-__global__ __launch_bounds__(kBlock) void tree_expand_select_kernel(Tree t, const float* __restrict__ lp1,
+__global__ __launch_bounds__(kBlock) __attribute__((amdgpu_num_sgpr(102))) void tree_expand_select_kernel(Tree t, const float* __restrict__ lp1,
                                                                     const float* __restrict__ lp2,
                                                                     const float* __restrict__ lpm,
                                                                     const float* __restrict__ values,
                                                                     const float* __restrict__ noise, int noise_stride,
-                                                                    float epsilon, int step, CapArrays cap,
-                                                                    ForcedArgs fa, GumbelArgs ga, SolverArgs sv,
-                                                                    ShapeArgs sh) {
+                                                                    float epsilon, int step, ArgsIf<CAP, CapArrays> cap_,
+                                                                    ArgsIf<FORCED, ForcedArgs> fa_,
+                                                                    ArgsIf<GUMBEL, GumbelArgs> ga_,
+                                                                    ArgsIf<SOLVER, SolverArgs> sv_,
+                                                                    ArgsIf<SHAPE, ShapeArgs> sh_) {
+    const CapArrays* cap = args_ptr<CapArrays>(cap_);
+    const ForcedArgs* fa = args_ptr<ForcedArgs>(fa_);
+    const GumbelArgs* ga = args_ptr<GumbelArgs>(ga_);
 #ifndef LZ_EXP_NO_TREE_PRIO
     __builtin_amdgcn_s_setprio(3);
 #endif
@@ -226,20 +236,25 @@
 #ifdef LZ_EXP_TREE_STAMPS
     const unsigned long long lz_t0 = __builtin_readcyclecounter();
 #endif
-    if (CAP && IS_ROOT && !cap_noise(cap, g)) noise = nullptr;
-    tree_expand<IS_ROOT, 0, SOLVER>(t, g, lane, lp1 + o * 36, lp2 + o * 36, lpm + o * 36, nullptr, values + o, noise,
-                                    noise_stride, epsilon, sc, &root, step, nullptr, nullptr, &sv LZ_TSTAMP_PASS);
+    if (CAP && IS_ROOT && !cap_noise(*cap, g)) noise = nullptr;
+    tree_expand<IS_ROOT, 0, SOLVER, ArgsViewed>(arg_view(t), g, lane, lp1 + o * 36, lp2 + o * 36, lpm + o * 36, nullptr, values + o, noise,
+                                    noise_stride, epsilon, sc, &root, step, nullptr, nullptr,
+                                                args_ptr<SolverArgs>(sv_) LZ_TSTAMP_PASS);
     __threadfence_block();
-    const bool gum_on = GUMBEL && (!CAP || cap_noise(cap, g));
-    if (GUMBEL && IS_ROOT && gum_on) { gumbel_root_step(t, g, lane, ga); __threadfence_block(); }
-    if (CAP && cap_spent(cap, g, step)) {
-        if (lane == 0) t.leaf_kind[g] = kLeafInactive;
+    const Tree& ts = arg_view(t);
+    const int gs = ArgsViewed::index(g);
+    const bool gum_on = GUMBEL && (!CAP || cap_noise(*cap, gs));
+    if (GUMBEL && IS_ROOT && gum_on) { gumbel_root_step(ts, gs, lane, *ga); __threadfence_block(); }
+    if (CAP && cap_spent(*cap, gs, step)) {
+        if (lane == 0) ts.leaf_kind[gs] = kLeafInactive;
         return;
     }
-    if (IS_ROOT) root = load_root_info(t, g);
+    if (IS_ROOT) root = load_root_info(ts, gs);
+    else root = unpark_root(root);
     LZ_TSTAMP(g, 7)
-    const double fk = FORCED && (!CAP || cap_noise(cap, g)) ? fa.k : 0.0;
-    tree_select<FORCED, GUMBEL, SOLVER, SHAPE>(t, g, lane, root, -1, -1, nullptr, fk, fa.count, &ga, gum_on, &sh LZ_TSTAMP_PASS);
+    const double fk = FORCED && (!CAP || cap_noise(*cap, gs)) ? fa->k : 0.0;
+    tree_select<FORCED, GUMBEL, SOLVER, SHAPE, ArgsViewed>(ts, gs, lane, root, -1, -1, nullptr, fk, FORCED ? fa->count : nullptr, ga,
+                                                           gum_on, args_ptr<ShapeArgs>(sh_) LZ_TSTAMP_PASS);
 #ifdef LZ_EXP_TREE_STAMPS
     LZ_TADD(g, 19, 1)
 #endif
@@ -251,7 +266,11 @@
                                                                           const float* __restrict__ lp2,
                                                                           const float* __restrict__ lpm,
                                                                           const float* __restrict__ values, int step,
-                                                                          CapArrays cap, ForcedArgs fa, GumbelArgs ga) {
+                                                                          ArgsIf<CAP, CapArrays> cap_,
+                                                                          ArgsIf<FORCED, ForcedArgs> fa_,
+                                                                          ArgsIf<GUMBEL, GumbelArgs> ga_) {
+    const CapArrays* cap = args_ptr<CapArrays>(cap_);
+    const ForcedArgs* fa = args_ptr<ForcedArgs>(fa_);
     __builtin_amdgcn_s_setprio(3);
     LZ_EXPAND_SCRATCH(sc);
     __shared__ int s_flag[kWavesPerBlock / 2];
@@ -266,24 +285,27 @@
     ptrdiff_t o = 0;
     if (COMPACT) o = (ptrdiff_t)(t.leaf_kind[g] == kLeafExpand ? t.live_row[g] : 0) - g;
     if (role == 0) {
-        tree_expand<false, 1>(t, g, lane, lp1 + o * 36, lp2 + o * 36, lpm + o * 36, nullptr, values + o, nullptr, 0, 0.f, sc,
-                              nullptr, step, flag);
+        tree_expand<false, 1, false, ArgsViewed>(t, g, lane, lp1 + o * 36, lp2 + o * 36, lpm + o * 36, nullptr, values + o, nullptr,
+                                                 0, 0.f, sc, nullptr, step, flag);
         __builtin_amdgcn_fence(__ATOMIC_RELEASE, "workgroup");
         if (lane == 0) *flag = kSplitExpanded;
     } else {
         RootInfo root;
         SplitInfo split;
-        tree_expand<false, 2>(t, g, lane, lp1 + o * 36, lp2 + o * 36, lpm + o * 36, nullptr, values + o, nullptr, 0, 0.f, sc,
-                              &root, step, flag, &split);
+        tree_expand<false, 2, false, ArgsViewed>(t, g, lane, lp1 + o * 36, lp2 + o * 36, lpm + o * 36, nullptr, values + o, nullptr,
+                                                 0, 0.f, sc, &root, step, flag, &split);
         __threadfence_block();
         split_wait(flag, kSplitInputsRead);
-        if (CAP && cap_spent(cap, g, step)) {
-            if (lane == 0) t.leaf_kind[g] = kLeafInactive;
+        root = unpark_root(root);
+        const Tree& ts = arg_view(t);
+        if (CAP && cap_spent(*cap, g, step)) {
+            if (lane == 0) ts.leaf_kind[g] = kLeafInactive;
             return;
         }
-        const double fk = FORCED && (!CAP || cap_noise(cap, g)) ? fa.k : 0.0;
-        const bool gum_on = GUMBEL && (!CAP || cap_noise(cap, g));
-        tree_select<FORCED, GUMBEL>(t, g, lane, root, split.wait_edge, split.nolegal_edge, flag, fk, fa.count, &ga, gum_on);
+        const double fk = FORCED && (!CAP || cap_noise(*cap, g)) ? fa->k : 0.0;
+        const bool gum_on = GUMBEL && (!CAP || cap_noise(*cap, g));
+        tree_select<FORCED, GUMBEL, false, false, ArgsViewed>(ts, g, lane, root, split.wait_edge, split.nolegal_edge, flag, fk,
+                                                              FORCED ? fa->count : nullptr, args_ptr<GumbelArgs>(ga_), gum_on);
     }
 }
 
diff --git a/liuzhou_amd/csrc/lz_search.hip b/liuzhou_amd/csrc/lz_search.hip
--- a/liuzhou_amd/csrc/lz_search.hip
+++ b/liuzhou_amd/csrc/lz_search.hip
@@ -71,17 +71,17 @@
             if (g >= t.B || (a.exp_mode & 3)) break;
             RootInfo root;
             if (s == 0) {
-                tree_expand<true>(t, g, ctx.lane, lp1, lp2, lpm, nullptr, values, a.noise, a.noise_stride, a.epsilon, sc, &root, s);
+                tree_expand<true, 0, false, ArgsReread>(arg_view(t), g, ctx.lane, lp1, lp2, lpm, nullptr, values, a.noise, a.noise_stride, a.epsilon, sc, &root, s);
                 if (a.sims > 0) {
                     __threadfence_block();
-                    root = load_root_info(t, g);
-                    tree_select(t, g, ctx.lane, root);
+                    root = load_root_info(arg_view(t), g);
+                    tree_select<false, false, false, false, ArgsReread>(arg_view(t), g, ctx.lane, root);
                 }
             } else {
-                tree_expand<false>(t, g, ctx.lane, lp1, lp2, lpm, nullptr, values, nullptr, 0, 0.f, sc, &root, s);
+                tree_expand<false, 0, false, ArgsReread>(arg_view(t), g, ctx.lane, lp1, lp2, lpm, nullptr, values, nullptr, 0, 0.f, sc, &root, s);
                 if (s < a.sims) {
                     __threadfence_block();
-                    tree_select(t, g, ctx.lane, root);
+                    tree_select<false, false, false, false, ArgsReread>(arg_view(t), g, ctx.lane, root);
                 }
             }
         }
diff --git a/liuzhou_amd/csrc/lz_tree_args.h b/liuzhou_amd/csrc/lz_tree_args.h
--- /dev/null
+++ b/liuzhou_amd/csrc/lz_tree_args.h
@@ -0,0 +1,30 @@
+#pragma once
+#include <stdint.h>
+
+#include <type_traits>
+
+namespace lz {
+
+struct CapArrays { const int* sim_budget; const uint8_t* root_noise; };
+struct ForcedArgs { double k; int* count; };
+struct SolverArgs { int* root_proven; int* count; };
+struct ShapeArgs { double fpu, fpu_root; const double* table; int flags, table_len; };
+struct GumbelArgs {
+    double c_visit, c_scale;
+    const float* g; const int* table;
+    float* gl; int* base; int* root_base; float* root_value; int* count;
+    int m, sims, stride;
+};
+
+struct EmptyArgs {
+    EmptyArgs() = default;
+    EmptyArgs(const CapArrays&) {}
+    EmptyArgs(const ForcedArgs&) {}
+    EmptyArgs(const SolverArgs&) {}
+    EmptyArgs(const ShapeArgs&) {}
+    EmptyArgs(const GumbelArgs&) {}
+};
+template <bool ON, class T> using ArgsIf = std::conditional_t<ON, T, EmptyArgs>;
+static_assert(std::is_empty<EmptyArgs>::value && std::is_trivially_copyable<EmptyArgs>::value, "EmptyArgs carries nothing");
+
+}
diff --git a/liuzhou_amd/csrc/lz_tree_dev.h b/liuzhou_amd/csrc/lz_tree_dev.h
--- a/liuzhou_amd/csrc/lz_tree_dev.h
+++ b/liuzhou_amd/csrc/lz_tree_dev.h
@@ -7,6 +7,7 @@
 #include "lz_rng.h"
 #include "lz_soa.h"
 #include "lz_symmetry.h"
+#include "lz_tree_args.h"
 #include "lz_wave.h"
 
 using namespace lz;
@@ -67,18 +68,10 @@
     int* leaf_sym; int* trace_sym; const int* sym_salt; const int64_t* sym_game; const int64_t* sym_ply;
     uint64_t sym_seed; int sym_mode, sym_fixed;
 };
-struct CapArrays { const int* sim_budget; const uint8_t* root_noise; };
-struct ForcedArgs { double k; int* count; };
-struct SolverArgs { int* root_proven; int* count; };
-struct ShapeArgs { double fpu, fpu_root; const double* table; int flags, table_len; };
 constexpr int kShapeFpu = 1, kShapeTable = 2;
 constexpr double kShapeFix = 1073741824.0;
-struct GumbelArgs {
-    double c_visit, c_scale;
-    const float* g; const int* table;
-    float* gl; int* base; int* root_base; float* root_value; int* count;
-    int m, sims, stride;
-};
+template <class T> __device__ __forceinline__ const T* args_ptr(const T& a) { return &a; }
+template <class T> __device__ __forceinline__ const T* args_ptr(const EmptyArgs&) { return nullptr; }
 
 typedef unsigned int u32x4 __attribute__((ext_vector_type(4)));
 __device__ __forceinline__ Edge load_edge(const Edge* p) {
@@ -161,6 +154,37 @@
     return 0.0;
 }
 
+
+template <class T>
+__device__ __forceinline__ const T& arg_view(const T& a) {
+    int z = 0;
+    asm volatile("" : "+s"(z));
+    return *reinterpret_cast<const T*>(reinterpret_cast<const char*>(&a) + z);
+}
+__device__ __forceinline__ int park(int x) { asm volatile("" : "+v"(x)); return x; }
+__device__ __forceinline__ int unpark(int x) { return __builtin_amdgcn_readfirstlane(x); }
+__device__ __forceinline__ uint64_t park(uint64_t x) {
+    return ((uint64_t)(uint32_t)park((int)(x >> 32)) << 32) | (uint32_t)park((int)(uint32_t)x);
+}
+__device__ __forceinline__ uint64_t unpark(uint64_t x) {
+    return ((uint64_t)(uint32_t)unpark((int)(x >> 32)) << 32) | (uint32_t)unpark((int)(uint32_t)x);
+}
+struct ArgsHeld {
+    template <class T> static __device__ __forceinline__ const T& again(const T& a) { return a; }
+    static __device__ __forceinline__ int index(int g) { return g; }
+    template <class T> static __device__ __forceinline__ T park(T x) { return x; }
+    template <class T> static __device__ __forceinline__ T unpark(T x) { return x; }
+};
+struct ArgsReread : ArgsHeld {
+    template <class T> static __device__ __forceinline__ const T& again(const T& a) { return arg_view(a); }
+    static __device__ __forceinline__ int index(int g) { asm volatile("" : "+s"(g)); return g; }
+};
+struct ArgsViewed {
+    template <class T> static __device__ __forceinline__ const T& again(const T& a) { return arg_view(a); }
+    static __device__ __forceinline__ int index(int g) { asm volatile("" : "+s"(g)); return g; }
+    template <class T> static __device__ __forceinline__ T park(T x) { return ::park(x); }
+    template <class T> static __device__ __forceinline__ T unpark(T x) { return ::unpark(x); }
+};
 
 __device__ __forceinline__ bool cap_spent(const CapArrays& c, int g, int step) {
     return c.sim_budget != nullptr && step >= c.sim_budget[g];
@@ -249,6 +273,12 @@
     return r;
 }
 
+__device__ __forceinline__ RootInfo unpark_root(const RootInfo& p) {
+    RootInfo r;
+    r.ne = unpark(p.ne); r.e0 = unpark(p.e0); r.visits = unpark(p.visits); r.player = unpark(p.player);
+    r.state.w0 = unpark(p.state.w0); r.state.w1 = unpark(p.state.w1); r.state.w2 = unpark(p.state.w2); r.state.w3 = unpark(p.state.w3);
+    return r;
+}
 constexpr int kSplitInputsRead = 1, kSplitExpanded = 2;
 __device__ __forceinline__ void split_wait(volatile int* flag, int phase) {
     while (*flag < phase) __builtin_amdgcn_s_sleep(1);
@@ -395,7 +425,7 @@
     return marks;
 }
 
-template <bool FORCED = false, bool GUMBEL = false, bool SOLVER = false, bool SHAPE = false>
+template <bool FORCED = false, bool GUMBEL = false, bool SOLVER = false, bool SHAPE = false, class ARGS = ArgsHeld>
 __device__ __forceinline__ void tree_select(const Tree& t, int g, int lane, const RootInfo& root, int wait_edge = -1,
                                             int nolegal_edge = -1, volatile int* flag = nullptr, double forced_k = 0.0,
                                             int* forced_count = nullptr, const GumbelArgs* gum = nullptr,
@@ -626,6 +656,8 @@
         if (depth >= t.path_cap - 1) break;
     }
     LZ_TSTAMP(g, 8)
+    const Tree& tl = ARGS::again(t);
+    const int gl = ARGS::index(g);
     Packed leaf_packed{};
     int src = -1;
     if (kind == kLeafExpand) {
@@ -634,25 +666,25 @@
         index_to_code(leaf.phase, leaf_action, kd, p, q2, ex);
         apply_legal(leaf, kd, p, q2);
         leaf_packed = pack(leaf);
-        if (t.share) {
-            src = pos_find(t, g, leaf_packed, t.n_nodes[g], lane);
+        if (tl.share) {
+            src = pos_find(tl, gl, leaf_packed, tl.n_nodes[gl], lane);
             if (src > 0) kind = kLeafShared;
         }
     }
     int sym = 0;
-    if (t.sym_mode != 0 && kind == kLeafExpand) {
-        sym = __builtin_amdgcn_readfirstlane(leaf_sym_for(t, g, leaf_packed));
+    if (tl.sym_mode != 0 && kind == kLeafExpand) {
+        sym = __builtin_amdgcn_readfirstlane(leaf_sym_for(tl, gl, leaf_packed));
         leaf_packed = sym_packed_wave(sym, leaf_packed, lane);
     }
     if (lane == 0) {
-        t.path_len[g] = depth;
-        t.leaf_kind[g] = kind;
-        t.leaf_value[g] = term_value;
-        t.leaf_edge[g] = leaf_edge;
-        t.leaf_parent[g] = node;
-        if (kind == kLeafExpand || kind == kLeafShared) t.leaf_state[g] = leaf_packed;
-        if (kind == kLeafShared) t.leaf_src[g] = src;
-        if (t.sym_mode != 0) t.leaf_sym[g] = sym;
+        tl.path_len[gl] = depth;
+        tl.leaf_kind[gl] = kind;
+        tl.leaf_value[gl] = term_value;
+        tl.leaf_edge[gl] = leaf_edge;
+        tl.leaf_parent[gl] = node;
+        if (kind == kLeafExpand || kind == kLeafShared) tl.leaf_state[gl] = leaf_packed;
+        if (kind == kLeafShared) tl.leaf_src[gl] = src;
+        if (tl.sym_mode != 0) tl.leaf_sym[gl] = sym;
     }
     LZ_TSTAMP(g, 9)
 }
@@ -666,7 +698,7 @@
     const ExpandScratch name = {name##_val[name##_wv], name##_act[name##_wv]}
 
 struct SplitInfo { int wait_edge, nolegal_edge; };
-template <bool IS_ROOT, int ROLE = 0, bool SOLVER = false>
+template <bool IS_ROOT, int ROLE = 0, bool SOLVER = false, class ARGS = ArgsHeld>
 __device__ __forceinline__ void tree_expand(const Tree& t, int g, int lane, const float* __restrict__ lp1,
                                             const float* __restrict__ lp2, const float* __restrict__ lpm,
                                             const float* __restrict__ priors220, const float* __restrict__ values,
@@ -689,17 +721,18 @@
     const int sym = (t.sym_mode != 0 && kind == kLeafExpand) ? (__builtin_amdgcn_readfirstlane(t.leaf_sym[g]) & 7) : 0;
     if (!IS_ROOT) {
         root = load_root_info(t, g);
-        plen_ld = t.path_len[g];
-        leaf_edge = t.leaf_edge[g];
-        leaf_parent = t.leaf_parent[g];
+        plen_ld = ARGS::park(t.path_len[g]);
+        leaf_edge = ARGS::park(t.leaf_edge[g]);
+        leaf_parent = ARGS::park(t.leaf_parent[g]);
         path_entry = lane < t.path_cap ? path[lane] : 0;
         root_w = t.root_W[g];
         leaf_value_ld = t.leaf_value[g];
     }
-    nn_ld = t.n_nodes[g];
-    ne_ld = t.n_edges[g];
+    nn_ld = ARGS::park(t.n_nodes[g]);
+    ne_ld = ARGS::park(t.n_edges[g]);
     const Packed eval_packed = leaf_packed;
     if (sym != 0) leaf_packed = sym_packed_wave(sym_inverse(sym), eval_packed, lane);
+    const Packed leaf_parked = {ARGS::park(leaf_packed.w0), ARGS::park(leaf_packed.w1), ARGS::park(leaf_packed.w2), ARGS::park(leaf_packed.w3)};
     const bool shared = !IS_ROOT && ROLE == 0 && kind == kLeafShared;
     value_ld = shared ? 0.f : values[g];
     const bool indexed = !IS_ROOT && ROLE != 2 && t.pos_index != nullptr;
@@ -711,7 +744,13 @@
         value_ld = t.node_value[(size_t)g * t.node_cap + src];
         src_begin = nodes[src].edge_begin;
     }
-    if (root_after != nullptr) *root_after = root;
+    if (root_after != nullptr) {
+        RootInfo pk;
+        pk.ne = ARGS::park(root.ne); pk.e0 = ARGS::park(root.e0); pk.visits = root.visits; pk.player = ARGS::park(root.player);
+        pk.state.w0 = ARGS::park(root.state.w0); pk.state.w1 = ARGS::park(root.state.w1);
+        pk.state.w2 = ARGS::park(root.state.w2); pk.state.w3 = ARGS::park(root.state.w3);
+        *root_after = pk;
+    }
     if (ROLE == 1) {
         asm volatile("s_waitcnt vmcnt(0)" ::: "memory");
         if (lane == 0) *flag = kSplitInputsRead;
@@ -766,7 +805,6 @@
         }
         return;
     }
-    const int plen = IS_ROOT ? 0 : plen_ld;
     double backup_value = 0.0;
     int sol = 0;
     bool sol_terminal = false;
@@ -783,15 +821,16 @@
         leaf_player = s.player;
         if (ROLE == 2) {
             backup_value = n == 0 ? -1.0 : (double)value_ld;
-            if (n == 0) split->nolegal_edge = leaf_edge; else split->wait_edge = leaf_edge;
+            if (n == 0) split->nolegal_edge = ARGS::unpark(leaf_edge); else split->wait_edge = ARGS::unpark(leaf_edge);
         } else if (n == 0) {
             backup_value = -1.0;
             if (lane == 0) {
+                const Tree& tz = ARGS::again(t);
                 if (IS_ROOT) {
-                    if (root_pending(t, g)) atomicSub(t.pool_stats + 2, 1);
-                    nodes[0].nedges = 0; t.root_terminal[g] = 1; t.root_init_value[g] = -1.f;
-                }
-                else atomicOr(&edges[(size_t)leaf_edge].n_info, (uint32_t)kInfoTerminal << 24);
+                    if (root_pending(tz, g)) atomicSub(tz.pool_stats + 2, 1);
+                    tz.nodes[(size_t)g * tz.node_cap].nedges = 0; tz.root_terminal[g] = 1; tz.root_init_value[g] = -1.f;
+                }
+                else atomicOr(&tz.edges[(size_t)leaf_edge].n_info, (uint32_t)kInfoTerminal << 24);
             }
             if (SOLVER && !IS_ROOT) { sol = 1; sol_terminal = true; }
         } else {
@@ -801,7 +840,7 @@
                 const int hc = sym != 0 ? sym_cell(sym, lane) : lane;
                 h1 = lp1[(size_t)g * 36 + hc]; h2 = lp2[(size_t)g * 36 + hc]; hm = lpm[(size_t)g * 36 + hc];
                 if (tracing) {
-                    float* th = t.trace_heads + tslot * 108;
+                    float* th = ARGS::again(t).trace_heads + tslot * 108;
                     th[hc] = h1; th[36 + hc] = h2; th[72 + hc] = hm;
                 }
             }
@@ -843,7 +882,7 @@
             if (tracing) {
 #pragma unroll
                 for (int it = 0; it < 4; ++it)
-                    if (lg[it]) t.trace_priors[tslot * 220 + it * kWave + lane] = val[it];
+                    if (lg[it]) ARGS::again(t).trace_priors[tslot * 220 + it * kWave + lane] = val[it];
             }
             if (IS_ROOT && noise != nullptr && n > 1) {
                 const float keep = (float)(1.0 - (double)epsilon);
@@ -865,12 +904,15 @@
                 cval[r] = k < n ? sc.val[k] : 0.f;
                 cact[r] = k < n ? sc.act[k] : 0;
             }
+            const Tree& ta = ARGS::again(t);
+            const int ga = ARGS::index(g);
+            Edge* edges_a = ta.edges;
             float psum = 0.f;
             if (shared) {
 #pragma unroll
                 for (int r = 0; r < 2; ++r) {
                     const int k = r * kWave + lane;
-                    cval[r] = k < n ? edges[(size_t)(src_begin + k)].P : 0.f;
+                    cval[r] = k < n ? edges_a[(size_t)(src_begin + k)].P : 0.f;
                 }
                 psum = 1.f;
             } else {
@@ -881,32 +923,33 @@
             LZ_TSTAMP(g, 3)
             int node_id = 0, e0 = 0;
             if (lane == 0) {
+                Node* nodes_a = ta.nodes + (size_t)ga * ta.node_cap;
                 e0 = ne_ld;
-                const int off = e0 & (t.chunk - 1);
-                if (off == 0 || off + n > t.chunk) e0 = take_chunk(t, g, IS_ROOT);
+                const int off = e0 & (ta.chunk - 1);
+                if (off == 0 || off + n > ta.chunk) e0 = take_chunk(ta, ga, IS_ROOT);
                 if (e0 >= 0) {
-                    t.n_edges[g] = e0 + n;
+                    ta.n_edges[ga] = e0 + n;
                     if (IS_ROOT) node_id = 0;
                     else {
-                        node_id = nn_ld; t.n_nodes[g] = node_id + 1;
-                        Edge& in = edges[(size_t)leaf_edge];
+                        node_id = nn_ld; ta.n_nodes[ga] = node_id + 1;
+                        Edge& in = edges_a[(size_t)leaf_edge];
                         in.child = node_id; in.cbegin = e0; in.cn = (uint8_t)n;
-                        nodes[node_id].state = leaf_packed;
-                        nodes[node_id].parent = leaf_parent;
-                        if (t.node_value != nullptr) t.node_value[(size_t)g * t.node_cap + node_id] = value_ld;
+                        nodes_a[node_id].state = leaf_parked;
+                        nodes_a[node_id].parent = leaf_parent;
+                        if (ta.node_value != nullptr) ta.node_value[(size_t)ga * ta.node_cap + node_id] = value_ld;
                         if (indexed && !shared && pw.first_empty < kWave)
-                            t.pos_index[(size_t)g * t.pos_slots + ((pw.base + (uint32_t)pw.first_empty) & ((uint32_t)t.pos_slots - 1u))] = node_id;
+                            ta.pos_index[(size_t)ga * ta.pos_slots + ((pw.base + (uint32_t)pw.first_empty) & ((uint32_t)ta.pos_slots - 1u))] = node_id;
                     }
-                    nodes[node_id].edge_begin = e0;
-                    nodes[node_id].nedges = n;
-                }
-                if (IS_ROOT) t.root_init_value[g] = value_ld;
+                    nodes_a[node_id].edge_begin = e0;
+                    nodes_a[node_id].nedges = n;
+                }
+                if (IS_ROOT) ta.root_init_value[ga] = value_ld;
             }
             e0 = __builtin_amdgcn_readfirstlane(e0);
             node_id = __builtin_amdgcn_readfirstlane(node_id);
             const int n_write = e0 >= 0 ? n : 0;
             LZ_TSTAMP(g, 4)
-            Edge* new_run = edges + (size_t)(e0 >= 0 ? e0 : 0);
+            Edge* new_run = edges_a + (size_t)(e0 >= 0 ? e0 : 0);
             uint8_t new_info[2] = {0, 0};
             for (int r = 0; r < (n_write > kWave ? 2 : 1); ++r) {
                 const int k = r * kWave + lane;
@@ -946,17 +989,22 @@
         if (sv->count != nullptr) sv->count[g] += 1;
     }
     if (IS_ROOT || ROLE == 1) return;
+    const int plen = ARGS::unpark(plen_ld);
     if (plen > 0) {
+        const Tree& tb = ARGS::again(t);
+        const int gb = ARGS::index(g);
+        Edge* edges_b = tb.edges;
+        const int* path_b = tb.path + (size_t)gb * tb.path_cap;
         int flips_above = 0;
         for (int hi = plen; hi > 0; hi -= kWave) {
             const int lo = hi > kWave ? hi - kWave : 0;
             const int j = lo + lane;
             const bool in = j < hi;
-            const uint32_t pe = !in ? 0u : (lo == 0 ? (uint32_t)path_entry : (uint32_t)path[j]);
+            const uint32_t pe = !in ? 0u : (lo == 0 ? (uint32_t)path_entry : (uint32_t)path_b[j]);
             const uint64_t F = __ballot(in && (pe & kPathFlip) != 0u);
             const int above = in ? __popcll(F >> (lane + 1)) : 0;
             if (in) {
-                Edge* e = &edges[(size_t)(pe & ~kPathFlip)];
+                Edge* e = &edges_b[(size_t)(pe & ~kPathFlip)];
                 const double v = ((above + flips_above) & 1) ? -backup_value : backup_value;
                 atomicAdd(&e->n_info, 1u);
                 unsafeAtomicAdd(&e->W, v);
@@ -965,16 +1013,16 @@
         }
         root.visits += 1;
         if (lane == 0) {
-            t.root_visits[g] = root.visits;
-            t.root_W[g] = root_w + ((flips_above & 1) ? -backup_value : backup_value);
+            tb.root_visits[gb] = root.visits;
+            tb.root_W[gb] = root_w + ((flips_above & 1) ? -backup_value : backup_value);
         }
         if (root_after != nullptr) root_after->visits = root.visits;
         if (SOLVER && sol != 0) {
             const uint8_t mark = (uint8_t)(kInfoProven | ((sol - 1) << 2));
-            if (!sol_terminal && lane == 0) atomicOr(&edges[(size_t)leaf_edge].n_info, (uint32_t)mark << 24);
+            if (!sol_terminal && lane == 0) atomicOr(&edges_b[(size_t)leaf_edge].n_info, (uint32_t)mark << 24);
             const uint8_t info_j = (uint8_t)((leaf_player < 0 ? kInfoWhite : 0) | (sol_terminal ? kInfoTerminal : mark));
-            const int marks = 1 + solver_climb(t, g, lane, *sv, path, plen - 1, leaf_edge, info_j, root);
-            if (sv->count != nullptr && lane == 0) sv->count[g] += marks;
+            const int marks = 1 + solver_climb(tb, gb, lane, *sv, path_b, plen - 1, ARGS::unpark(leaf_edge), info_j, root);
+            if (sv->count != nullptr && lane == 0) sv->count[gb] += marks;
             __builtin_amdgcn_fence(__ATOMIC_ACQ_REL, "agent");
         }
     }
```

Measured after the change: 12370 (median of 3 runs). No clear change (+0.0%).
